# exoclime/HELIOS

Hardware: AMD Instinct MI355X
Metric: rad-conv iterations/sec x (lambda-bins x layers) (higher is better)
Workload: dtype f64; 1 GPU; BASELINE config 2: single column, 10 000 bins x 100 layers, premixed corr-k, isotropic scattering; nbin=10000, nlayer=100, ny=20, species=0, columns_per_gpu=1, columns_total=1, loop=radiative, parallelism=columns sharded, 1 per GPU

## Files before the change

helios_amd/csrc/rt_coef_kernel.inc:

```
template <int ROWS, int COEF_TPB>
__global__ void __launch_bounds__(64 * COEF_TPB) HX_COEF_KERNEL(KArgs a HX_PLANE_ARG) {
    using CT = HX_PLANE_T;
    extern __shared__ __align__(16) double smem[];
    const int col = blockIdx.y;
    if (a.done[col]) return;
    const int wave = threadIdx.x >> 6, lane = threadIdx.x & 63;
    const int ntiles = a.nblk_x * a.nparts * a.NW;
    const int TS = COEF_TPB * a.S;
    const int TSP = TS;
    const int NBX = a.coef_nbx;
    double* sh_lay = smem;
    double* sh_int = sh_lay + (size_t)a.L * TSP;
    double* sh_ray = sh_int + (size_t)a.I * TSP;
    double* sh_mu = sh_ray + (size_t)a.H * NBX;
    double* sh_dc = sh_mu + a.H;
    const size_t ncl = a.cloud_lds ? (size_t)a.H * NBX : 0;
    double* sh_g0 = sh_dc + a.H;
    double* sh_cab = sh_g0 + ncl;
    double* sh_csc = sh_cab + ncl;
    int* c_of_q = (int*)(sh_csc + ncl);
    int* x_of_q = c_of_q + TS;
    const size_t nc = (size_t)a.Y * a.X;
    const size_t wgI = nc * a.I;
    const int x_base = (blockIdx.x * COEF_TPB) / (a.NW * a.nparts) * a.nxb;
    for (int q = threadIdx.x; q < TS; q += blockDim.x) {
        const int tl = blockIdx.x * COEF_TPB + q / a.S, s_in_wave = q % a.S;
        int c = -1, xq = x_base;
        if (tl < ntiles) {
            const int wv = tl % a.NW, part = (tl / a.NW) % a.nparts, bx = tl / (a.NW * a.nparts);
            const int s_local = wv * a.S + s_in_wave;
            const int xl = s_local / a.ypb, yl = s_local - xl * a.ypb;
            const int x = bx * a.nxb + xl, y = part * a.ypb + yl;
            if (s_local < a.G && x < a.X) { c = y + a.Y * x; xq = x; }
        }
        c_of_q[q] = c;
        x_of_q[q] = xq;
    }
    {
        const double* mml = a.mmm_lay + (size_t)col * a.I;
        const double* mmi = a.mmm_int + (size_t)col * a.I;
        const double* dcu = a.dcol_u + (size_t)col * a.L;
        const double* dcl = a.dcol_l + (size_t)col * a.L;
        const double* pint = a.p_int + (size_t)col * a.I;
        const double grav = a.colpar[col].g;
        for (int h = threadIdx.x; h < a.H; h += blockDim.x) {
            if (a.iso) {
                sh_mu[h] = mml[h];
                sh_dc[h] = (pint[h] - pint[h + 1]) / grav;
            } else {
                const int i = h >> 1, ii = i + (h & 1);
                sh_mu[h] = (mmi[ii] + mml[i]) / 2.0;
                sh_dc[h] = (h & 1) ? dcu[i] : dcl[i];
            }
        }
        for (int t = threadIdx.x; t < a.H * NBX; t += blockDim.x) {
            const int xs = t / a.H, h = t - xs * a.H, x = min(x_base + xs, a.X - 1);
            const size_t src = ((size_t)col * a.X + x) * a.H + h;
            sh_ray[(size_t)h * NBX + xs] = a.half_ray[src];
            if (a.cloud_lds) {
                sh_g0[(size_t)h * NBX + xs] = a.half_g0[src];
                sh_cab[(size_t)h * NBX + xs] = a.half_cab[src];
                sh_csc[(size_t)h * NBX + xs] = a.half_csc[src];
            }
        }
    }
    __syncthreads();
    {
        const int q0 = threadIdx.x % TS, nrun = blockDim.x / TS, run = threadIdx.x / TS;
        const int cq = c_of_q[q0];
        if (a.from_table) {
            const size_t sp = nc, st = nc * a.npress;
            const double* ktable = a.coltab[col].k;
            for (int pass = 0; pass < (a.iso ? 1 : 2); pass++) {
                const int nlev = pass == 0 ? a.L : a.I;
                const TPIndex* tp = (pass == 0 ? a.tp_lay : a.tp_int) + (size_t)col * a.I;
                double* dst = pass == 0 ? sh_lay : sh_int;
                const int per = (nlev + nrun - 1) / nrun;
                const int l0 = run * per, l1 = min(nlev, l0 + per);
                int ktd = -1, ktu = -1, kpd = -1, kpu = -1;
                double c00 = 0, c01 = 0, c10 = 0, c11 = 0;
                TPIndex knext = tp[min(l0, nlev - 1)];
                for (int lev = l0; lev < l1; lev++) {
                    double v = 0.0;
                    const TPIndex k = knext;
                    knext = tp[min(lev + 1, nlev - 1)];
                    if (cq >= 0) {
                        if (k.tdown != ktd || k.tup != ktu || k.pdown != kpd || k.pup != kpu) {
                            const double* t0 = ktable + (size_t)cq + st * k.tdown;
                            const double* t1 = ktable + (size_t)cq + st * k.tup;
                            c00 = t0[sp * k.pdown];
                            c01 = t0[sp * k.pup];
                            c10 = t1[sp * k.pdown];
                            c11 = t1[sp * k.pup];
                            ktd = k.tdown; ktu = k.tup; kpd = k.pdown; kpu = k.pup;
                        }
                        v = blend_tp(c00, c01, c10, c11, k, false);
                    }
                    dst[(size_t)lev * TSP + q0] = v;
                }
            }
        } else {
            const double* opl = a.opac_wg_lay + col * wgI;
            const double* opi = a.opac_wg_int + col * wgI;
            for (int lev = run; lev < a.L; lev += nrun)
                sh_lay[(size_t)lev * TSP + q0] = cq >= 0 ? opl[(size_t)cq + nc * lev] : 0.0;
            if (!a.iso)
                for (int lev = run; lev < a.I; lev += nrun)
                    sh_int[(size_t)lev * TSP + q0] = cq >= 0 ? opi[(size_t)cq + nc * lev] : 0.0;
        }
    }
    __syncthreads();
    const int tl = blockIdx.x * COEF_TPB + wave;
    if (tl >= ntiles) return;
    const int j = lane % a.k, q = wave * a.S + lane / a.k;
    const int c = c_of_q[q], x = x_of_q[q], xs = x - x_base;
    const bool valid = c >= 0;
    const hx_rt_column cp = a.colpar[col];
    CT* ctile = HX_PLANES + col * a.coef_col + (size_t)tl * a.nplane * ROWS * 64;
    const double nmu = -cp.mu_star;
    const bool plain = a.clouds != 1 && a.scat_corr != 1 && a.g_0 == 0.0 && a.dir_beam != 1;
    const double* Fd = a.F_dir_wg + col * wgI;
    const double* Fc = a.Fc_dir_wg + col * wgI;
    auto beam_at_node = [&](int n) -> double {
        if (!(a.dir_beam == 1 && valid && n <= a.H)) return 0.0;
        if (a.iso) return Fd[(size_t)c + nc * n];
        return (n & 1) ? Fc[(size_t)c + nc * (n >> 1)] : Fd[(size_t)c + nc * (n >> 1)];
    };
    double F_here = beam_at_node(j * ROWS), F_above = beam_at_node(j * ROWS + 1);
    bool scatters = true;
    if (a.matrix) {
        bool mine = false;
#pragma unroll 1
        for (int r = 0; r < ROWS; r++) {
            const int h = j * ROWS + r;
            if (valid && h < a.H) {
                const int i = a.iso ? h : h >> 1;
                const bool lower = a.iso || (h & 1) == 0;
                const int ii = lower ? i : i + 1;
                double ray = 0.0, csc = 0.0, cab = 0.0;
                if (a.cloud_lds) {
                    cab = sh_cab[(size_t)h * NBX + xs];
                    csc = sh_csc[(size_t)h * NBX + xs];
                } else if (a.clouds == 1) {
                    const size_t src = ((size_t)col * a.X + x) * a.H + h;
                    cab = a.half_cab[src];
                    csc = a.half_csc[src];
                }
                if (a.scat == 1) ray = sh_ray[(size_t)h * NBX + xs];
                const double o_l = sh_lay[(size_t)i * TSP + q], o_i = a.iso ? o_l : sh_int[(size_t)ii * TSP + q];
                const double kap = a.iso ? o_l : (lower ? (o_i + o_l) / 2.0 : (o_l + o_i) / 2.0);
                mine = mine || single_scat_albedo(ray + csc, kap * sh_mu[h] + cab, a.w_0_limit) > a.w_0_scat_limit;
            }
        }
        const unsigned long long votes = __ballot(mine);
        const unsigned long long group = a.k >= 64 ? ~0ull : ((1ull << a.k) - 1ull) << (lane - j);
        scatters = (votes & group) != 0ull;
        if (valid && j == 0) a.trigger[col * nc + c] = scatters ? 1 : 0;
    }
    for (int r = 0; r < ROWS; r++) {
        const int h = j * ROWS + r;
        double alpha = 1.0, beta = 0.0, up = 0.0, vp = 0.0, dd = 0.0, du = 0.0;
        const double Fbot = F_here, Ftop = F_above;
        F_here = F_above;
        F_above = beam_at_node(h + 2);
        if (valid && h < a.H) {
            const int i = a.iso ? h : h >> 1;
            const bool lower = a.iso || (h & 1) == 0;
            const int ii = lower ? i : i + 1;
            double g0 = a.g_0, ray = 0.0, csc = 0.0, cab = 0.0;
            if (a.cloud_lds) {
                g0 = sh_g0[(size_t)h * NBX + xs];
                cab = sh_cab[(size_t)h * NBX + xs];
                csc = sh_csc[(size_t)h * NBX + xs];
            } else if (a.clouds == 1) {
                const size_t src = ((size_t)col * a.X + x) * a.H + h;
                g0 = a.half_g0[src];
                cab = a.half_cab[src];
                csc = a.half_csc[src];
            }
            if (a.scat == 1) ray = sh_ray[(size_t)h * NBX + xs];
            const double o_l = sh_lay[(size_t)i * TSP + q], o_i = a.iso ? o_l : sh_int[(size_t)ii * TSP + q];
            const double kap = a.iso ? o_l : (lower ? (o_i + o_l) / 2.0 : (o_l + o_i) / 2.0);
            const double mu = sh_mu[h], dcol = sh_dc[h];
            const double w0 = single_scat_albedo(ray + csc, kap * mu + cab, a.w_0_limit);
            const double dtau_gas = dcol * (kap + ray / mu);
            const double dtau = plain ? dtau_gas : dtau_gas + dcol * (cab + csc) / mu;
            const Slab s = plain ? slab_coeffs_plain(w0, dtau, a.epsi)
                                 : slab_coeffs(w0, dtau, g0, a.epsi, a.epsi2, cp.mu_star, a.scat_corr, a.i2s, a.dir_beam == 1);
            if (a.diag != nullptr && a.dir_beam == 1) {
                const int nlim = (fabs(s.Gp) >= 1e8 ? 1 : 0) + (fabs(s.Gm) >= 1e8 ? 1 : 0);
                if (nlim) atomicAdd(a.diag + HX_DIAG_G_LIMITED, (unsigned long long)nlim);
            }
            double invM = 1.0 / s.M;
            alpha = s.P * invM;
            beta = -s.N * invM;
            double K = 2.0 * HX_PI * a.epsi * (1.0 - w0) / (s.E - w0);
            double u, v;
            if (!scatters) {
                alpha = s.trans;
                beta = 0.0;
                invM = 1.0;
                K = 2.0 * HX_PI * a.epsi;
                if (a.iso || dtau < a.dtau_limit) {
                    u = v = (1.0 - s.trans) / 2.0;
                } else {
                    const double gq = a.epsi * (s.trans - 1.0) / dtau;
                    u = 1.0 + gq;
                    v = -s.trans - gq;
                }
            } else if (a.iso || dtau < a.dtau_limit) {
                u = v = (s.N + s.M - s.P) / 2.0;
            } else {
                const double qq = (plain ? a.epsi : a.epsi / (s.E * (1.0 - w0 * g0))) * (s.P - s.M + s.N) / dtau;
                u = (s.M + s.N) + qq;
                v = -s.P - qq;
            }
            up = K * u * invM;
            vp = K * v * invM;
            if (a.dir_beam == 1 && scatters) {
                const double dn = Fbot / nmu * (s.Gm * s.M + s.Gp * s.N) - Ftop / nmu * s.Gm * s.P;
                const double upw = Ftop / nmu * (s.Gm * s.N + s.Gp * s.M) - Fbot / nmu * s.P * s.Gp;
                dd = dmin(0.0, dn) * invM;
                du = dmin(0.0, upw) * invM;
            }
            if (h == 0) {
                a.boaK[col * nc + c] = scatters ? (1.0 - w0) / (s.E - w0) : 1.0;
                a.Fdir0[col * nc + c] = a.dir_beam == 1 ? (a.F_dir_wg + col * wgI)[c] : 0.0;
            }
        }
        const size_t off = plane_off(r, lane, ROWS);
        if constexpr (sizeof(CT) == sizeof(double)) {
            __builtin_nontemporal_store(alpha, ctile + 0 * ROWS * 64 + off);
            __builtin_nontemporal_store(beta, ctile + 1 * ROWS * 64 + off);
            __builtin_nontemporal_store(up, ctile + 2 * ROWS * 64 + off);
            if (a.has_vp) __builtin_nontemporal_store(vp, ctile + (size_t)a.pl_vp * ROWS * 64 + off);
        } else {
            __builtin_nontemporal_store(plane0_code(alpha, beta), ctile + 0 * ROWS * 64 + off);
            __builtin_nontemporal_store(plane1_code(beta), ctile + 1 * ROWS * 64 + off);
            __builtin_nontemporal_store((CT)up, ctile + 2 * ROWS * 64 + off);
            if (a.has_vp) __builtin_nontemporal_store((CT)(up + vp), ctile + (size_t)a.pl_vp * ROWS * 64 + off);
        }
        if (a.dir_beam == 1) {
            __builtin_nontemporal_store((CT)dd, ctile + (size_t)a.pl_dd * ROWS * 64 + off);
            __builtin_nontemporal_store((CT)du, ctile + (size_t)(a.pl_dd + 1) * ROWS * 64 + off);
        }
    }
}
```

helios_amd/csrc/rt_fused.h:

```cpp
#pragma once
#include <string>
#include <vector>

#include "hx_common.h"

namespace hx {

struct TileGeom {
    int k, ROWS, S;
    int nxb, ypb, nparts, G, NW, threads;
    int nblk_x;
    int nblk;
    int nplane;
    int has_vp, pl_vp, pl_dd;
    size_t tile_rows;
    size_t coef_elems_per_col, flux_elems_per_col;
};

struct Species {
    double* pretab = nullptr;
    double* scat_cross = nullptr;
    double* vmr_tab = nullptr;
    bool vmr_from_tab = false;
    double weight = 0.0;
    int is_h2o = 0, is_cia = 0, in_mu = 1;
    bool absorbing = false, scattering = false;
};

struct TableSet {
    const double *k, *scat_cross, *meanmass;
};

struct MieTable {
    const double *lam, *scat, *absorb;
    int nw, nr;
};

struct ProfileEntry {
    std::string name;
    hipEvent_t e0, e1;
};

}

struct hx_rt {
    hx_context* ctx;
    hx_rt_dims d;
    hx_rt_flags f;
    std::vector<hx_rt_column> cols;
    int X, Y, L, I, H, C, nsweep;
    hx::TileGeom g;
    bool have_grid = false, have_tables = false, have_planck = false, refreshed = false;
    bool keep_down = false;
    bool opac_stale = false;
    void* tp_lay = nullptr;
    void* tp_int = nullptr;
    double *T_lay_ref = nullptr, *T_int_ref = nullptr;
    int nchunk;
    int coef_tpb = 4;
    hipError_t shmem_rc = hipSuccess;
    bool cloud_lds = true;
    bool serpentine = false;
    unsigned flux_launches = 0;
    double state_cache_mb = 0;
    bool generic_scans = false;
    bool conv_shmem_raised = false;
    bool coef_shmem_raised = false;

    double *interwave = nullptr, *deltawave = nullptr, *wave = nullptr, *gauss_y = nullptr,
           *gauss_w = nullptr, *ktemp = nullptr, *kpress = nullptr;
    std::vector<hx::TableSet> tables;
    std::vector<int> col_table;
    hx::TableSet* coltab = nullptr;
    hx::TableSet* coltab_ref = nullptr;
    double* planck_grid = nullptr;
    std::vector<hx::Species> species;
    void* species_dev = nullptr;
    int* abs_list = nullptr;
    int nabs = 0;
    bool species_dev_stale = true;
    double *fac_lay = nullptr, *fac_int = nullptr;
    double *spec_lay = nullptr, *spec_int = nullptr;
    double *sc_spec_lay = nullptr, *sc_spec_int = nullptr;

    hx_rt_column* colpar = nullptr;
    double *p_lay = nullptr, *p_int = nullptr, *dcol_u = nullptr, *dcol_l = nullptr;
    double *T_lay = nullptr, *T_int = nullptr;
    double *surf_albedo = nullptr, *starflux = nullptr, *Bstar = nullptr;
    double *opac_wg_lay = nullptr, *opac_wg_int = nullptr;
    double *scat_cross_lay = nullptr, *scat_cross_int = nullptr;
    double *mmm_lay = nullptr, *mmm_int = nullptr;
    double *cl_abs_lay = nullptr, *cl_abs_int = nullptr, *cl_sc_lay = nullptr, *cl_sc_int = nullptr,
           *cl_g0_lay = nullptr, *cl_g0_int = nullptr, *g0_tot_lay = nullptr, *g0_tot_int = nullptr;
    double *half_ray = nullptr, *half_g0 = nullptr, *half_cab = nullptr, *half_csc = nullptr;
    double *vmr_lay = nullptr, *vmr_int = nullptr;
    double *delta_z = nullptr, *z_lay = nullptr;
    double *dtau_u = nullptr, *dtau_l = nullptr;
    double *F_dir_wg = nullptr, *Fc_dir_wg = nullptr;
    double* F_dir_band_n = nullptr;
    double* Bn = nullptr;
    double* coef = nullptr;
    float* coef32 = nullptr;
    int coef_bytes = 8;
    double* Utile = nullptr;
    double* Dtile = nullptr;
    double *U0 = nullptr, *boaK = nullptr, *Fdir0 = nullptr;
    double *F_down_band_n = nullptr, *F_up_band_n = nullptr;
    double* tot_part = nullptr;
    double *F_up_tot = nullptr, *F_down_tot = nullptr, *F_net = nullptr, *F_net_diff = nullptr;
    double *T_store = nullptr, *prefactor = nullptr;
    double *F_add_heat_lay = nullptr, *F_add_heat_sum = nullptr, *F_smooth = nullptr,
           *F_smooth_sum = nullptr, *c_p_lay = nullptr;
    int *abort_flags = nullptr, *conv_count = nullptr, *done = nullptr, *iters_done = nullptr;
    double *kappa_lay = nullptr, *kappa_int = nullptr, *dampara = nullptr;
    int *conv_unstable = nullptr, *conv_layer = nullptr, *marked_red = nullptr;
    double *entr_temp = nullptr, *entr_press = nullptr, *entr_kappa = nullptr, *entr_c_p = nullptr;
    int entr_ntemp = 0, entr_npress = 0;
    double* add_heat_dens = nullptr;
    bool has_heating = false;

    std::vector<hx::MieTable> mie;
    hx::MieTable* mie_dev = nullptr;
    double* cloud_spec = nullptr;
    int cloud_ndecks = 0;
    double* cloud_stage = nullptr;
    int* cloud_stage_index = nullptr;
    int cloud_stage_nr = 0;

    bool matrix = false;
    int* trigger = nullptr;
    bool matrix_keep_state = false;
    int* zero_flags = nullptr;
    int* iter_dev = nullptr;
    int iter_dev_expected = -1;
    hipGraphExec_t iter_graph = nullptr;
    hipGraphExec_t decade_graph = nullptr;
    long long iter_graph_replays = 0, decade_graph_replays = 0;
    long long iter_graph_builds = 0, decade_graph_builds = 0;
    long long graph_gen = 1, iter_graph_gen = 0, decade_graph_gen = 0;
    long long solve_serial = 1, matrix_tiles_serial = 0;
    int use_graph = -1;
    std::vector<char> have_albedo;

    bool profiling = false;
    std::vector<hx::ProfileEntry> prof;
    std::vector<std::pair<std::string, std::pair<double, int>>> prof_acc;
    std::vector<void*> allocs;
};
```

helios_amd/csrc/rt_fused.hip:

```cpp
#include "rt_kernels.h"
#include "rt_species.h"

#include <algorithm>
#include <cmath>

using namespace hx;

namespace {

int rt_fail(hx_rt* rt, int code, const char* msg) { return hx_fail(rt->ctx, code, "%s", msg); }

template <class T>
int dev_alloc(hx_rt* rt, T** p, size_t n, bool zero = true) {
    void* q = nullptr;
    if (n == 0) n = 1;
    hipError_t e = hipMalloc(&q, n * sizeof(T));
    if (e != hipSuccess)
        return hx_fail(rt->ctx, -(int)e, "hipMalloc of %zu bytes failed: %s", n * sizeof(T),
                       hipGetErrorString(e));
    if (zero) {
        e = hipMemsetAsync(q, 0, n * sizeof(T), rt->ctx->stream);
        if (e != hipSuccess) return hx_fail(rt->ctx, -(int)e, "hipMemset failed");
    }
    rt->allocs.push_back(q);
// ... 118 lines not shown
    a.U0 = rt->U0; a.boaK = rt->boaK; a.Fdir0 = rt->Fdir0;
    a.dtau_u = rt->dtau_u; a.dtau_l = rt->dtau_l;
    a.F_down_band_n = rt->F_down_band_n; a.F_up_band_n = rt->F_up_band_n; a.tot_part = rt->tot_part;
    a.F_up_tot = rt->F_up_tot; a.F_down_tot = rt->F_down_tot; a.F_net = rt->F_net;
    a.coef_col = g.coef_elems_per_col; a.flux_col = g.flux_elems_per_col;
    a.done = rt->done;
    a.coltab = rt->coltab; a.ktemp = rt->ktemp; a.kpress = rt->kpress;
    a.tp_lay = (const TPIndex*)rt->tp_lay; a.tp_int = (const TPIndex*)rt->tp_int;
    a.ntemp = rt->d.ntemp; a.npress = rt->d.npress; a.from_table = 0;
    a.iter_dev = rt->iter_dev;
    return a;
}

struct ProfScope {
    hx_rt* rt;
    hipEvent_t e0 = nullptr, e1 = nullptr;
    const char* name;
    ProfScope(hx_rt* r, const char* n) : rt(r), name(n) {
        if (!rt->profiling) return;
        (void)hipEventCreate(&e0);
        (void)hipEventCreate(&e1);
        (void)hipEventRecord(e0, rt->ctx->stream);
    }
    ~ProfScope() {
        if (!rt->profiling) return;
        (void)hipEventRecord(e1, rt->ctx->stream);
        rt->prof.push_back({name, e0, e1});
        if (rt->prof.size() > 8192) flush(rt);
    }
    static void flush(hx_rt* rt) {
        for (auto& p : rt->prof) {
            (void)hipEventSynchronize(p.e1);
            float ms = 0;
            (void)hipEventElapsedTime(&ms, p.e0, p.e1);
            bool found = false;
            for (auto& acc : rt->prof_acc)
                if (acc.first == p.name) {
                    acc.second.first += ms;
                    acc.second.second += 1;
                    found = true;
                }
            if (!found) rt->prof_acc.push_back({p.name, {ms, 1}});
            (void)hipEventDestroy(p.e0);
            (void)hipEventDestroy(p.e1);
        }
        rt->prof.clear();
    }
};

size_t flux_shmem_bytes(hx_rt* rt) {
    const TileGeom& g = rt->g;
    return ((size_t)g.nxb * (rt->H + 3) + (size_t)g.nxb * 2 * rt->I + (size_t)g.ypb * g.nxb * 2 * rt->I) *
           sizeof(double);
}

#define DISPATCH_ROWS(fn, rt, a)                  \
    switch ((rt)->g.ROWS) {                       \
        case 1: fn<1>(rt, a); break;              \
        case 2: fn<2>(rt, a); break;              \
        case 3: fn<3>(rt, a); break;              \
        case 4: fn<4>(rt, a); break;              \
        case 5: fn<5>(rt, a); break;              \
        case 6: fn<6>(rt, a); break;              \
        case 7: fn<7>(rt, a); break;              \
        case 8: fn<8>(rt, a); break;              \
        case 9: fn<9>(rt, a); break;              \
        case 10: fn<10>(rt, a); break;            \
        case 11: fn<11>(rt, a); break;            \
        case 12: fn<12>(rt, a); break;            \
        case 13: fn<13>(rt, a); break;            \
        case 14: fn<14>(rt, a); break;            \
        case 15: fn<15>(rt, a); break;            \
        case 20: fn<20>(rt, a); break;            \
        case 24: fn<24>(rt, a); break;            \
        case 28: fn<28>(rt, a); break;            \
        case 32: fn<32>(rt, a); break;            \
        default: fn<16>(rt, a); break;            \
    }

template <int ROWS, int K, bool MATRIX>
void flux_kernel(hx_rt* rt, const FluxArgs* f) {
    const size_t shmem = flux_shmem_bytes(rt);
    if (!f) {
        rt->shmem_rc = hipFuncSetAttribute((const void*)k_rt_flux<ROWS, K, MATRIX>, hipFuncAttributeMaxDynamicSharedMemorySize,
                                           (int)shmem);
        return;
    }
    hipLaunchKernelGGL(HIP_KERNEL_NAME(k_rt_flux<ROWS, K, MATRIX>), dim3(rt->g.nblk_x, rt->C), dim3(rt->g.threads), shmem,
                       rt->ctx->stream, *f);
}

template <int ROWS, bool MATRIX>
void flux_method(hx_rt* rt, const FluxArgs* f) {
    const int k = rt->g.k;
    const bool generic = rt->generic_scans;
    if constexpr (ROWS > 16) {
        (void)k; (void)generic;
        flux_kernel<ROWS, 64, MATRIX>(rt, f);
    } else {
        if (k == 16 && !generic) flux_kernel<ROWS, 16, MATRIX>(rt, f);
        else if (k == 32 && !generic) flux_kernel<ROWS, 32, MATRIX>(rt, f);
        else if (k == 64 && !generic) flux_kernel<ROWS, 64, MATRIX>(rt, f);
        else flux_kernel<ROWS, 0, MATRIX>(rt, f);
    }
}

template <int ROWS>
void flux_rows(hx_rt* rt, const FluxArgs* f) {
    if (rt->matrix) flux_method<ROWS, true>(rt, f);
    else flux_method<ROWS, false>(rt, f);
}

void launch_flux(hx_rt* rt, const KArgs& a) {
    const TileGeom& g = rt->g;
    FluxArgs f;
    memset(&f, 0, sizeof(f));
    f.X = a.X; f.Y = a.Y; f.L = a.L; f.I = a.I; f.H = a.H;
    f.k = a.k; f.nxb = a.nxb; f.ypb = a.ypb; f.nparts = a.nparts; f.G = a.G; f.NW = a.NW;
    f.dir_beam = a.dir_beam; f.nsweep = a.nsweep; f.keep_down = a.keep_down; f.has_vp = a.has_vp;
    f.pl_vp = a.pl_vp; f.pl_dd = a.pl_dd; f.nplane = a.nplane; f.iso = a.iso;
#ifdef HX_PROFILING
    static const int debug_skip = [] { const char* e = getenv("HELIOS_RT_DEBUG_SKIP"); return e ? atoi(e) : 0; }();
    f.debug_skip = debug_skip;
#endif
    f.Kconst = a.Kconst;
    f.trigger = a.trigger;
    f.keep_up = rt->matrix_keep_state ? 1 : 0;
    f.colpar = a.colpar;
    f.Bn = a.Bn; f.coef = a.coef; f.U0_in = a.U0; f.boaK = a.boaK; f.Fdir0 = a.Fdir0;
    f.surf_albedo = a.surf_albedo; f.gauss_w = a.gauss_w;
    f.Utile = a.Utile; f.Dtile = a.Dtile; f.U0 = a.U0; f.F_down_band_n = a.F_down_band_n;
    f.F_up_band_n = a.F_up_band_n;
    f.coef_col = a.coef_col; f.flux_col = a.flux_col;
    f.done = a.done;
    f.reverse = rt->serpentine ? (rt->flux_launches++ & 1) : 0;
    f.cache_state_from = INT_MAX;
    if (rt->serpentine && rt->state_cache_mb > 0) {
        const double per_wg = (double)g.nparts * g.NW * g.ROWS * 64 * sizeof(double);
        const long long total = (long long)g.nblk_x * rt->C;
        const long long keep = (long long)(rt->state_cache_mb * 1048576.0 / per_wg);
        f.cache_state_from = (int)std::max(0LL, total - keep);
    }
    if (rt->matrix) {
        f.reverse = 0;
        f.cache_state_from = INT_MAX;
    }
    if (rt->coef32) {
        launch_flux_f32(rt, f, dim3(g.nblk_x, rt->C), flux_shmem_bytes(rt));
        return;
    }
    DISPATCH_ROWS(flux_rows, rt, &f);
}

template <int ROWS, int TPB>
void launch_coef_tpb(hx_rt* rt, KArgs a) {
    const TileGeom& g = rt->g;
    const int ntiles = g.nblk_x * g.nparts * g.NW;
    const int TS = TPB * g.S, TSP = TS;
    const int NBX = g.nxb * ((TPB - 1) / (g.NW * g.nparts) + 2);
    a.coef_nbx = NBX;
    size_t shmem = ((size_t)(rt->L + rt->I) * TSP + (size_t)rt->H * (NBX + 2)) * sizeof(double) + 2 * TS * sizeof(int);
    const size_t cloud_image = 3 * (size_t)rt->H * NBX * sizeof(double);
    a.cloud_lds = a.clouds == 1 && rt->cloud_lds && shmem + cloud_image <= 80 * 1024;
    if (a.cloud_lds) shmem += cloud_image;
    if (rt->coef32) {
        launch_coef_f32(rt, a, TPB, dim3((ntiles + TPB - 1) / TPB, rt->C), shmem);
        return;
    }
    if (shmem > 64 * 1024 && !rt->coef_shmem_raised) {
        (void)hipFuncSetAttribute((const void*)k_rt_coef<ROWS, TPB>, hipFuncAttributeMaxDynamicSharedMemorySize,
                                  (int)shmem);
        rt->coef_shmem_raised = true;
    }
    hipLaunchKernelGGL(HIP_KERNEL_NAME(k_rt_coef<ROWS, TPB>), dim3((ntiles + TPB - 1) / TPB, rt->C), dim3(64 * TPB),
                       shmem, rt->ctx->stream, a);
}
template <int ROWS>
void launch_coef(hx_rt* rt, const KArgs& a) {
    switch (rt->coef_tpb) {
        case 1: launch_coef_tpb<ROWS, 1>(rt, a); break;
        case 2: launch_coef_tpb<ROWS, 2>(rt, a); break;
        case 8:
            if constexpr (ROWS <= 16) { launch_coef_tpb<ROWS, 8>(rt, a); break; }
            [[fallthrough]];
        default: launch_coef_tpb<ROWS, 4>(rt, a); break;
    }
}

size_t coef_shmem_bytes(const hx_rt* rt, int tpb) {
    const TileGeom& g = rt->g;
    const int TS = tpb * g.S;
    const int NBX = g.nxb * ((tpb - 1) / (g.NW * g.nparts) + 2);
    return ((size_t)(rt->L + rt->I) * TS + (size_t)rt->H * (NBX + 2)) * sizeof(double) + 2 * TS * sizeof(int);
}

int set_flux_shmem_limits(hx_rt* rt) {
    const size_t shmem = flux_shmem_bytes(rt);
    if (shmem > 160 * 1024) return rt_fail(rt, HX_E_UNSUPPORTED, "workgroup LDS demand exceeds 160 KiB");
    if (shmem <= 64 * 1024) return 0;
    if (rt->coef_bytes == 4) {
        HX_HIP(rt->ctx, raise_flux_shmem_f32(rt, (int)shmem));
        return 0;
    }
    DISPATCH_ROWS(flux_rows, rt, nullptr);
    HX_HIP(rt->ctx, rt->shmem_rc);
    return 0;
}

}

extern "C" {

int hx_rt_struct_sizes(int* dims_size, int* flags_size, int* column_size) {
    if (dims_size) *dims_size = (int)sizeof(hx_rt_dims);
    if (flags_size) *flags_size = (int)sizeof(hx_rt_flags);
    if (column_size) *column_size = (int)sizeof(hx_rt_column);
    return 0;
}

static int rt_create_into(hx_rt* rt, hx_context* ctx, const hx_rt_dims* dims, const hx_rt_flags* flags,
                          const hx_rt_column* columns);

int hx_rt_create(hx_context* ctx, const hx_rt_dims* dims, const hx_rt_flags* flags,
                 const hx_rt_column* columns, hx_rt** out_rt) {
    if (!ctx || !dims || !flags || !columns || !out_rt) return HX_E_ARG;
    *out_rt = nullptr;
    HX_REQUIRE(ctx, dims->nbin > 0 && dims->ny > 0 && dims->nlayer >= 1 && dims->ncol > 0, HX_E_ARG,
               "bad dimensions");
    HX_REQUIRE(ctx, dims->plancktable_dim >= 10 && dims->plancktable_step > 0, HX_E_ARG,
               "bad Planck-table dimensions");
    HX_HIP(ctx, hipSetDevice(ctx->device));
    hx_rt* rt = new hx_rt();
    const int rc_create = rt_create_into(rt, ctx, dims, flags, columns);
    if (rc_create) {
        hx_rt_destroy(rt);
        return rc_create;
    }
    *out_rt = rt;
    return 0;
}

static int rt_create_into(hx_rt* rt, hx_context* ctx, const hx_rt_dims* dims, const hx_rt_flags* flags,
                          const hx_rt_column* columns) {
    rt->ctx = ctx;
    rt->d = *dims;
    rt->f = *flags;
    rt->cols.assign(columns, columns + dims->ncol);
    rt->X = dims->nbin; rt->Y = dims->ny; rt->L = dims->nlayer; rt->I = rt->L + 1;
    rt->H = flags->iso ? rt->L : 2 * rt->L;
    rt->C = dims->ncol;
    rt->have_albedo.assign(dims->ncol, 0);
    rt->col_table.assign(dims->ncol, 0);
    RT_ALLOC(rt->iter_dev, 2);
    rt->nsweep = (flags->singlewalk ? 1000 : 3) * (flags->scat ? 1 : 0) + 1;
#ifdef HX_PROFILING
    if (const char* e = getenv("HELIOS_RT_DEBUG_NSWEEP")) rt->nsweep = atoi(e);
#endif
    if (const char* e = getenv("HELIOS_RT_MATRIX"))
        return hx_fail(ctx, HX_E_ARG, "HELIOS_RT_MATRIX=%s: the knob is retired (the matrix method has one solver); unset it", e);
    rt->matrix = flags->matrix != 0;
    rt->matrix_keep_state = rt->matrix && flags->debug == 1;
    if (!choose_geometry(rt->H, rt->Y, rt->X, rt->C, flags->dir_beam, flags->scat_corr, rt->g, rt->matrix ? 1 : 0))
        return hx_fail(ctx, HX_E_UNSUPPORTED, "fused path supports nlayer <= 1024 (2048 isothermal layers); use the per-stage API");
    rt->nchunk = std::max(1, std::min(512, std::max((rt->X + 47) / 48, std::min(32, (rt->X + 7) / 8))));
    if (const char* e = getenv("HELIOS_RT_GENERIC_SCANS")) rt->generic_scans = atoi(e) != 0;
    rt->coef_bytes = flags->coef_fp32 && !rt->matrix && coef_fp32_tiling(rt->g.ROWS, rt->g.k, rt->generic_scans) ? 4 : 8;
    if (const char* e = getenv("HELIOS_RT_CLOUD_LDS")) rt->cloud_lds = atoi(e) != 0;
    rt->coef_tpb = std::max(1, std::min(8, 16 / std::max(1, rt->g.S)));
    if (const char* e = getenv("HELIOS_RT_COEF_TPB")) rt->coef_tpb = atoi(e);
    if (rt->coef_tpb != 1 && rt->coef_tpb != 2 && !(rt->coef_tpb == 8 && rt->g.ROWS <= 16)) rt->coef_tpb = 4;
    while (rt->coef_tpb > 1 && coef_shmem_bytes(rt, rt->coef_tpb) > 150 * 1024) rt->coef_tpb /= 2;
    if (coef_shmem_bytes(rt, rt->coef_tpb) > 160 * 1024)
        return hx_fail(ctx, HX_E_UNSUPPORTED, "k_rt_coef's staging of one tile exceeds the 160 KiB of LDS");
    if (const char* e = getenv("HELIOS_RT_NCHUNK")) rt->nchunk = std::max(1, std::min(4096, atoi(e)));
    {
        const double state_mb = (double)rt->C * rt->g.flux_elems_per_col * sizeof(double) / 1048576.0;
        const double between_mb = (double)rt->C * rt->X * ((rt->H + 3) + 4.0 * rt->I) * sizeof(double) / 1048576.0;
        rt->serpentine = state_mb >= 64.0 && between_mb <= 64.0;
        rt->state_cache_mb = rt->serpentine ? 240.0 : 0.0;
    }
    if (const char* e = getenv("HELIOS_RT_SERPENTINE")) rt->serpentine = atoi(e) != 0;
    if (const char* e = getenv("HELIOS_RT_STATE_CACHE_MB")) rt->state_cache_mb = atof(e);
    rt->species.resize(dims->nspecies > 0 ? dims->nspecies : 0);
    int rc = set_flux_shmem_limits(rt);
    if (rc) return rc;

    const size_t X = rt->X, Y = rt->Y, L = rt->L, I = rt->I, C = rt->C, nc = X * Y;
    RT_ALLOC(rt->interwave, X + 1); RT_ALLOC(rt->deltawave, X); RT_ALLOC(rt->wave, X);
    RT_ALLOC(rt->gauss_y, Y); RT_ALLOC(rt->gauss_w, Y);
    RT_ALLOC(rt->ktemp, dims->ntemp); RT_ALLOC(rt->kpress, dims->npress);
    RT_ALLOC(rt->planck_grid, (size_t)(dims->plancktable_dim + 1) * X);
    RT_ALLOC(rt->colpar, C);
    RT_ALLOC(rt->coltab, C);
    RT_ALLOC(rt->coltab_ref, C);
    RT_ALLOC(rt->p_lay, C * L); RT_ALLOC(rt->p_int, C * I); RT_ALLOC(rt->dcol_u, C * L);
    RT_ALLOC(rt->dcol_l, C * L); RT_ALLOC(rt->T_lay, C * (L + 1)); RT_ALLOC(rt->T_int, C * I);
    RT_ALLOC(rt->surf_albedo, C * X); RT_ALLOC(rt->starflux, C * X); RT_ALLOC(rt->Bstar, C * X);
    RT_ALLOC(rt->opac_wg_lay, C * nc * I); RT_ALLOC(rt->opac_wg_int, C * nc * I);
    RT_ALLOC(rt->scat_cross_lay, C * X * I); RT_ALLOC(rt->scat_cross_int, C * X * I);
    RT_ALLOC(rt->mmm_lay, C * I); RT_ALLOC(rt->mmm_int, C * I);
    RT_ALLOC(rt->cl_abs_lay, C * X * I); RT_ALLOC(rt->cl_abs_int, C * X * I);
    RT_ALLOC(rt->cl_sc_lay, C * X * I); RT_ALLOC(rt->cl_sc_int, C * X * I);
    if (flags->clouds) {
        RT_ALLOC(rt->cl_g0_lay, C * X * I); RT_ALLOC(rt->cl_g0_int, C * X * I);
    }
    RT_ALLOC(rt->g0_tot_lay, C * X * I); RT_ALLOC(rt->g0_tot_int, C * X * I);
    RT_ALLOC(rt->half_ray, C * X * rt->H);
    if (flags->clouds) {
        RT_ALLOC(rt->half_g0, C * X * rt->H); RT_ALLOC(rt->half_cab, C * X * rt->H); RT_ALLOC(rt->half_csc, C * X * rt->H);
    }
    if (dims->nspecies > 0) {
        RT_ALLOC(rt->vmr_lay, C * dims->nspecies * I); RT_ALLOC(rt->vmr_int, C * dims->nspecies * I);
        RT_ALLOC(rt->spec_lay, nc * I); RT_ALLOC(rt->spec_int, nc * I);
        RT_ALLOC(rt->sc_spec_lay, X * I); RT_ALLOC(rt->sc_spec_int, X * I);
    }
    RT_ALLOC(rt->delta_z, C * L); RT_ALLOC(rt->z_lay, C * L);
    if (flags->dir_beam) {
        RT_ALLOC(rt->dtau_u, C * nc * L); RT_ALLOC(rt->dtau_l, C * nc * L);
        RT_ALLOC(rt->F_dir_wg, C * nc * I); RT_ALLOC(rt->Fc_dir_wg, C * nc * I);
    }
    RT_ALLOC(rt->F_dir_band_n, C * X * I);
    RT_ALLOC(rt->Bn, C * X * (rt->H + 3));
    if (rt->matrix) RT_ALLOC(rt->trigger, C * nc);
    if (rt->coef_bytes == 4) RT_ALLOC(rt->coef32, C * rt->g.coef_elems_per_col);
    else RT_ALLOC(rt->coef, C * rt->g.coef_elems_per_col);
    RT_ALLOC(rt->Utile, C * rt->g.flux_elems_per_col);
    RT_ALLOC(rt->U0, C * nc); RT_ALLOC(rt->boaK, C * nc); RT_ALLOC(rt->Fdir0, C * nc);
    RT_ALLOC(rt->F_down_band_n, C * X * I); RT_ALLOC(rt->F_up_band_n, C * X * I);
    RT_ALLOC(rt->tot_part, C * rt->nchunk * 2 * I);
    RT_ALLOC(rt->F_up_tot, C * I); RT_ALLOC(rt->F_down_tot, C * I); RT_ALLOC(rt->F_net, C * I);
    RT_ALLOC(rt->F_net_diff, C * L);
    RT_ALLOC(rt->T_store, C * (L + 1)); RT_ALLOC(rt->prefactor, C * (L + 1));
    RT_ALLOC(rt->F_add_heat_lay, C * L); RT_ALLOC(rt->F_add_heat_sum, C * L);
    RT_ALLOC(rt->F_smooth, C * L); RT_ALLOC(rt->F_smooth_sum, C * L); RT_ALLOC(rt->c_p_lay, C * L);
    RT_ALLOC(rt->abort_flags, C * (L + 1)); RT_ALLOC(rt->conv_count, C); RT_ALLOC(rt->done, C);
    RT_ALLOC(rt->kappa_lay, C * L); RT_ALLOC(rt->kappa_int, C * I); RT_ALLOC(rt->dampara, C);
    RT_ALLOC(rt->conv_unstable, C * (L + 1)); RT_ALLOC(rt->conv_layer, C * (L + 1)); RT_ALLOC(rt->marked_red, C * (L + 1));
    RT_ALLOC(rt->iters_done, C);
    {
        TPIndex* t1 = nullptr; TPIndex* t2 = nullptr;
        RT_ALLOC(t1, C * I); RT_ALLOC(t2, C * I);
        rt->tp_lay = t1; rt->tp_int = t2;
    }
    RT_ALLOC(rt->T_lay_ref, C * (L + 1)); RT_ALLOC(rt->T_int_ref, C * I);
    if (dims->nspecies > 0) {
        SpeciesDev* sd = nullptr;
        RT_ALLOC(sd, (size_t)dims->nspecies);
        rt->species_dev = sd;
        RT_ALLOC(rt->abs_list, (size_t)dims->nspecies);
        RT_ALLOC(rt->fac_lay, C * I * dims->nspecies); RT_ALLOC(rt->fac_int, C * I * dims->nspecies);
    }
    return h2d(rt, rt->colpar, rt->cols.data(), C * sizeof(hx_rt_column));
}

int hx_rt_destroy(hx_rt* rt) {
    if (!rt) return 0;
    if (rt->ctx) (void)hipStreamSynchronize(rt->ctx->stream);
    ProfScope::flush(rt);
    if (rt->iter_graph) (void)hipGraphExecDestroy(rt->iter_graph);
    if (rt->decade_graph) (void)hipGraphExecDestroy(rt->decade_graph);
    for (void* p : rt->allocs) (void)hipFree(p);
    delete rt;
    return 0;
}

#define RT_NEED_LOOP(rt)                                                                                             \
    do {                                                                                                             \
        if ((rt)->L < 2)                                                                                             \
            return hx_fail((rt)->ctx, HX_E_UNSUPPORTED, "%s: the batch has %d layer; refresh and iterations need at " \
                           "least 2", __func__, (rt)->L);                                                            \
    } while (0)

static inline void rt_touch(hx_rt* rt) {
    rt->graph_gen++;
    rt->solve_serial++;
}

int hx_rt_set_grid(hx_rt* rt, const double* opac_interwave, const double* opac_deltawave,
                   const double* opac_wave, const double* gauss_y, const double* gauss_weight,
                   const double* ktemp, const double* kpress) {
    if (!rt) return HX_E_ARG;
    rt_touch(rt);
    int rc = 0;
    rc |= h2d(rt, rt->interwave, opac_interwave, (rt->X + 1) * 8);
    rc |= h2d(rt, rt->deltawave, opac_deltawave, rt->X * 8);
    rc |= h2d(rt, rt->wave, opac_wave, rt->X * 8);
    rc |= h2d(rt, rt->gauss_y, gauss_y, rt->Y * 8);
    rc |= h2d(rt, rt->gauss_w, gauss_weight, rt->Y * 8);
    rc |= h2d(rt, rt->ktemp, ktemp, rt->d.ntemp * 8);
    rc |= h2d(rt, rt->kpress, kpress, rt->d.npress * 8);
    rt->have_grid = rc == 0;
    return rc;
}

static int for_cols(hx_rt* rt, int col, int* c0, int* c1);

static int upload_coltab(hx_rt* rt, int c0, int c1) {
    std::vector<TableSet> m(c1 - c0);
    for (int c = c0; c < c1; c++) m[c - c0] = rt->tables[rt->col_table[c]];
    return h2d(rt, rt->coltab + c0, m.data(), m.size() * sizeof(TableSet));
}

static int new_table_set(hx_rt* rt) {
    const size_t ntp = (size_t)rt->d.ntemp * rt->d.npress;
    const size_t n[3] = {ntp * rt->X * rt->Y, ntp * rt->X, ntp};
    double* p[3] = {nullptr, nullptr, nullptr};
    for (int i = 0; i < 3; i++)
        if (const int rc = dev_alloc(rt, &p[i], n[i])) {
            const std::string why = rt->ctx->err;
            return hx_fail(rt->ctx, rc, "premixed table set %d: %zu sets of %zu bytes each were asked for on this "
                           "device, the last one did not fit (%s)", (int)rt->tables.size(), rt->tables.size() + 1,
                           (n[0] + n[1] + n[2]) * 8, why.c_str());
        }
    rt->tables.push_back({p[0], p[1], p[2]});
    return rt->tables.size() == 1 ? upload_coltab(rt, 0, rt->C) : 0;
}

int hx_rt_set_premixed_tables(hx_rt* rt, const double* opac_k, const double* opac_scat_cross,
                              const double* opac_meanmass) {
    if (!rt) return HX_E_ARG;
    rt_touch(rt);
    HX_REQUIRE(rt->ctx, rt->d.nspecies == 0, HX_E_STATE, "object was created for on-the-fly mixing");
    const size_t ntp = (size_t)rt->d.ntemp * rt->d.npress;
    if (rt->tables.empty()) {
        int rc0 = new_table_set(rt);
        if (rc0) return rc0;
    }
    const TableSet& t = rt->tables[0];
    int rc = 0;
    rc |= h2d(rt, (void*)t.k, opac_k, ntp * rt->X * rt->Y * 8);
    rc |= h2d(rt, (void*)t.scat_cross, opac_scat_cross, ntp * rt->X * 8);
    rc |= h2d(rt, (void*)t.meanmass, opac_meanmass, ntp * 8);
    rt->have_tables = rc == 0;
    return rc;
}

int hx_rt_add_premixed_tables(hx_rt* rt, const double* opac_k, const double* opac_scat_cross, const double* opac_meanmass,
                              int* out_index) {
// ... 242 lines not shown
}

int hx_rt_set_convergence_limit(hx_rt* rt, int col, double limit) {
    if (!rt) return HX_E_ARG;
    rt_touch(rt);
    int c0, c1, rc = for_cols(rt, col, &c0, &c1);
    if (rc) return rc;
    for (int c = c0; c < c1; c++) {
        rt->cols[c].rad_convergence_limit = limit;
        rc |= h2d(rt, &rt->colpar[c], &rt->cols[c], sizeof(hx_rt_column));
    }
    return rc;
}


int hx_rt_build_planck_table(hx_rt* rt, int energy_correction) {
    if (!rt) return HX_E_ARG;
    rt_touch(rt);
    HX_REQUIRE(rt->ctx, rt->have_grid, HX_E_STATE, "hx_rt_set_grid first");
    hx_context* ctx = rt->ctx;
    const int X = rt->X, dim = rt->d.plancktable_dim, step = rt->d.plancktable_step;
    int rc = hx_plancktable(ctx, rt->planck_grid, rt->interwave, rt->deltawave, X, rt->cols[0].T_star,
                            dim, step);
    if (rc) return rc;
    for (int c = 0; c < rt->C; c++) {
        const double Ts = rt->cols[c].T_star;
        double* brow = rt->Bstar + (size_t)c * X;
        double* sflux = rt->starflux + (size_t)c * X;
        rc = hx_internal_planck_star_row(ctx, brow, rt->interwave, rt->deltawave, X, Ts);
        if (rc) return rc;
        if (energy_correction == 1 && Ts > 10) {
            rc = hx_corr_inc_energy(ctx, brow, sflux, rt->deltawave, rt->f.real_star, X, Ts, 0);
            if (rc) return rc;
        }
        if (rt->f.real_star == 1) {
            std::vector<double> tmp(X);
            rc = hx_d2h(ctx, tmp.data(), sflux, X * 8);
            if (rc) return rc;
            for (auto& v : tmp) v = v / HX_PI;
            rc = h2d(rt, brow, tmp.data(), X * 8);
            if (rc) return rc;
        }
        if (c == 0) {
            rc = hx_d2d(ctx, rt->planck_grid + (size_t)dim * X, brow, X * 8);
            if (rc) return rc;
        }
    }
    rt->have_planck = true;
    return 0;
}

static int upload_species_table(hx_rt* rt) {
    if (!rt->species_dev_stale) return 0;
    const int S = rt->d.nspecies;
    std::vector<SpeciesDev> sd(S);
    std::vector<int> abs;
    for (int s = 0; s < S; s++) {
        const Species& sp = rt->species[s];
        sd[s] = SpeciesDev{sp.pretab, sp.scat_cross, sp.vmr_from_tab ? sp.vmr_tab : nullptr, sp.weight, sp.absorbing ? 1 : 0,
                           sp.scattering ? 1 : 0,
                           sp.is_h2o ? 1 : 0, (rt->f.kcoeff_mixing_ro && !sp.is_cia && rt->Y != 1) ? 1 : 0,
                           sp.in_mu, 0};
        if (sp.absorbing) abs.push_back(s);
    }
    int rc = h2d(rt, rt->species_dev, sd.data(), S * sizeof(SpeciesDev));
    if (!rc && !abs.empty()) rc = h2d(rt, rt->abs_list, abs.data(), abs.size() * sizeof(int));
    rt->nabs = (int)abs.size();
    rt->species_dev_stale = rc != 0;
    return rc;
}

extern "C++" int hx::launch_mix_species(hx_context* ctx, MixArgs m, const int* abs_list, int nabs_all) {
    const long long npair = (long long)m.C * (m.L + m.I) * m.X;
    if (npair <= 0) return 0;
    static const int waves = [] { const char* e = getenv("HELIOS_RT_MIX_WAVES"); return e ? atoi(e) : 256 * 16 * 48; }();
    const int grid = (int)std::min(npair, (long long)waves);
    static const int extra_lds = [] { const char* e = getenv("HELIOS_RT_MIX_EXTRA_LDS"); return e ? atoi(e) : 0; }();
    for (int first = 0; first == 0 || first < nabs_all; first += MIX_MAX_ABSORBERS) {
        m.abs_list = abs_list + first;
        m.nabs = std::min(MIX_MAX_ABSORBERS, nabs_all - first);
        m.carry_on = first > 0 ? 1 : 0;
        k_rt_mix_species<<<grid, 64, extra_lds, ctx->stream>>>(m);
        HX_LAUNCH_CHECK(ctx);
    }
    return 0;
}

static int refresh_species(hx_rt* rt) {
    hx_context* ctx = rt->ctx;
    int rc = upload_species_table(rt);
    if (rc) return rc;
    MixArgs m;
    m.X = rt->X; m.Y = rt->Y; m.L = rt->L; m.I = rt->I; m.C = rt->C; m.S = rt->d.nspecies;
    m.ntemp = rt->d.ntemp; m.npress = rt->d.npress; m.nabs = rt->nabs; m.carry_on = 0;
    m.sp = (const SpeciesDev*)rt->species_dev; m.abs_list = rt->abs_list;
    m.T_lay = rt->T_lay; m.T_int = rt->T_int; m.p_lay = rt->p_lay; m.p_int = rt->p_int;
    m.vmr_lay = rt->vmr_lay; m.vmr_int = rt->vmr_int;
    m.ktemp = rt->ktemp; m.kpress = rt->kpress; m.gauss_w = rt->gauss_w; m.gauss_y = rt->gauss_y; m.wave = rt->wave;
    m.mmm_lay = rt->mmm_lay; m.mmm_int = rt->mmm_int;
    m.tp_lay = (TPIndex*)rt->tp_lay; m.tp_int = (TPIndex*)rt->tp_int;
    m.fac_lay = rt->fac_lay; m.fac_int = rt->fac_int;
    m.opac_wg_lay = rt->opac_wg_lay; m.opac_wg_int = rt->opac_wg_int;
    m.scat_lay = rt->scat_cross_lay; m.scat_int = rt->scat_cross_int;
    m.done = rt->done; m.diag = ctx->diag;
    k_rt_species_prep<<<dim3(hx_cdiv(rt->I, 64), rt->C), 64, 0, ctx->stream>>>(m);
    HX_LAUNCH_CHECK(ctx);
    {
        ProfScope ps(rt, "add_to_mixed_opac");
        rc = launch_mix_species(ctx, m, rt->abs_list, rt->nabs);
        if (rc) return rc;
    }
    {
        ProfScope ps(rt, "mixed_scat");
        k_rt_scat_species<<<dim3(hx_cdiv(rt->X, 256), rt->L + rt->I, rt->C), 256, 0, ctx->stream>>>(m);
        HX_LAUNCH_CHECK(ctx);
    }
    return 0;
}

int hx_rt_refresh(hx_rt* rt) {
    if (!rt) return HX_E_ARG;
    RT_NEED_LOOP(rt);
    hx_context* ctx = rt->ctx;
    rt->solve_serial++;
    HX_REQUIRE(ctx, rt->have_grid && rt->have_tables && rt->have_planck, HX_E_STATE,
               "set grid, tables and build the Planck table first");
    HX_REQUIRE(ctx, !rt->matrix || std::all_of(rt->have_albedo.begin(), rt->have_albedo.end(), [](char v) { return v != 0; }),
               HX_E_STATE, "the matrix method needs a surface albedo (> 0) for every column of the batch");
    const int X = rt->X, Y = rt->Y, L = rt->L, I = rt->I, C = rt->C;
    const size_t nc = (size_t)X * Y;
    int rc = 0;
    if (rt->d.nspecies > 0) {
        bool any_ro = false;
        for (const Species& sp : rt->species) any_ro = any_ro || (sp.absorbing && rt->f.kcoeff_mixing_ro && !sp.is_cia);
        if (Y != ro::NY && Y != 1 && any_ro)
            return hx_fail(ctx, HX_E_RO_NY, "random-overlap mixing needs ny == 20 or 1 (got %d)", Y);
        HX_REQUIRE(ctx, Y <= ro::NY, HX_E_UNSUPPORTED, "on-the-fly mixing in the fused path holds at most 20 Gauss points");
        int nabs = 0;
        for (const Species& sp : rt->species) nabs += sp.absorbing ? 1 : 0;
        (void)nabs;
    }
    KArgs a = make_args(rt);
    rt->iter_dev_expected = -1;
    {
        ProfScope ps(rt, "rt_nodes");
        dim3 grid(hx_cdiv(X, 32), hx_cdiv(rt->H + 3, 32), C);
        k_rt_nodes<<<grid, 256, 0, ctx->stream>>>(a);
        HX_LAUNCH_CHECK(ctx);
    }
    ProfScope ps_all(rt, "refresh_total");
    bool fused_lookup = rt->d.nspecies == 0 && !rt->f.dir_beam;
    if (const char* e = getenv("HELIOS_RT_FUSED_LOOKUP")) fused_lookup = fused_lookup && atoi(e) != 0;
    rt->opac_stale = fused_lookup;
    if (rt->d.nspecies == 0) {
        k_rt_tp_index<<<dim3(hx_cdiv(I, 64), C), 64, 0, ctx->stream>>>(a, (TPIndex*)rt->tp_lay, (TPIndex*)rt->tp_int);
        k_rt_scat_interp<<<dim3(hx_cdiv(X, 256), I, C), 256, 0, ctx->stream>>>(a, rt->scat_cross_lay, rt->scat_cross_int);
        k_rt_mmm_table<<<dim3(hx_cdiv(I, 64), C), 64, 0, ctx->stream>>>(a, rt->mmm_lay, rt->mmm_int);
        HX_LAUNCH_CHECK(ctx);
        if (fused_lookup) {
            k_rt_keep_ref_T<<<dim3(hx_cdiv(I + 1, 64), C), 64, 0, ctx->stream>>>(a, rt->T_lay_ref, rt->T_int_ref, rt->coltab_ref);
        } else {
            ProfScope ps(rt, "opac_interpol");
            const int chunks = (int)std::min<long long>(hx_cdiv((long long)nc, 256), 1024);
            k_rt_opac_table<<<dim3(chunks, I, C), 256, 0, ctx->stream>>>(a, rt->opac_wg_lay, rt->opac_wg_int);
        }
        HX_LAUNCH_CHECK(ctx);
    } else {
        rc = refresh_species(rt);
        if (rc) return rc;
    }
    if (rt->f.clouds) {
        k_rt_total_g0<<<dim3(hx_cdiv(X, 256), I, C), 256, 0, ctx->stream>>>(a, rt->cl_g0_lay, rt->cl_g0_int,
                                                                          rt->g0_tot_lay, rt->g0_tot_int);
        HX_LAUNCH_CHECK(ctx);
    }
    k_rt_delta_z<<<dim3(hx_cdiv(L, 64), C), 64, 0, ctx->stream>>>(a, rt->delta_z);
    k_rt_height<<<C, 64, 0, ctx->stream>>>(rt->p_lay, rt->delta_z, rt->z_lay, L, rt->f.planet_type_gas, (size_t)L, rt->done);
    HX_LAUNCH_CHECK(ctx);
    if (rt->has_heating) {
        k_rt_heating<<<C, 64, 0, ctx->stream>>>(rt->add_heat_dens, rt->delta_z, rt->F_add_heat_lay,
                                                rt->F_add_heat_sum, L, rt->done);
        HX_LAUNCH_CHECK(ctx);
    }
    if (rt->f.dir_beam) {
        ProfScope ps(rt, "direct_beam");
        k_rt_dtau_halves<<<dim3(hx_cdiv((long long)nc, 256), L, C), 256, 0, ctx->stream>>>(a);
        HX_LAUNCH_CHECK(ctx);
        rc = hx_internal_fdir_noniso_batch(ctx, rt->F_dir_wg, rt->f.iso ? nullptr : rt->Fc_dir_wg, rt->Bstar, rt->dtau_u, rt->dtau_l,
                                           rt->z_lay, rt->colpar, rt->done, C, rt->f.dir_beam,
                                           rt->f.geom_zenith_corr, I, X, Y);
        if (rc) return rc;
        k_rt_fdir_band<<<dim3(hx_cdiv(X, 32), hx_cdiv(I, 32), C), 256, 0, ctx->stream>>>(rt->F_dir_wg, rt->F_dir_band_n,
                                                                           rt->gauss_w, X, Y, I, rt->done);
        HX_LAUNCH_CHECK(ctx);
    }
    {
        ProfScope ps(rt, "rt_coef");
        k_rt_half_bands<<<dim3(hx_cdiv(X, 32), hx_cdiv(rt->H, 32), C), 256, 0, ctx->stream>>>(a);
        HX_LAUNCH_CHECK(ctx);
        a.from_table = fused_lookup ? 1 : 0;
        DISPATCH_ROWS(launch_coef, rt, a);
        HX_LAUNCH_CHECK(ctx);
    }
    rt->refreshed = true;
    return 0;
}

namespace { int kappa_cp_from_table(hx_rt* rt, bool refresh_T_int); }

static int count_negative_fluxes(hx_rt* rt) {
    const size_t n = (size_t)rt->C * rt->g.flux_elems_per_col;
    int rc = hx_internal_count_negative(rt->ctx, rt->Utile, n, HX_DIAG_NEG_UP);
    if (!rc && rt->keep_down && rt->Dtile) rc = hx_internal_count_negative(rt->ctx, rt->Dtile, n, HX_DIAG_NEG_DOWN);
    return rc;
}

static int spectral_fluxes(hx_rt* rt, const KArgs& a) {
    {
        ProfScope ps(rt, rt->matrix ? "matrix_solve" : "rt_flux");
        launch_flux(rt, a);
        HX_LAUNCH_CHECK(rt->ctx);
    }
    return rt->f.debug == 1 ? count_negative_fluxes(rt) : 0;
}

static int rt_step_kernels(hx_rt* rt, int itervalue, int step_temperature, bool nodes_done) {
    hx_context* ctx = rt->ctx;
    rt->solve_serial++;
    KArgs a = make_args(rt);
    if (!nodes_done) {
        ProfScope ps(rt, "rt_nodes");
        dim3 grid(hx_cdiv(rt->X, 32), hx_cdiv(rt->H + 3, 32), rt->C);
        k_rt_nodes<<<grid, 256, 0, ctx->stream>>>(a);
        HX_LAUNCH_CHECK(ctx);
    }
    {
        int rc = spectral_fluxes(rt, a);
        if (rc) return rc;
    }
    {
        ProfScope ps(rt, "rt_totals_a");
        k_rt_totals_a<<<dim3(rt->nchunk, rt->C), 256, 0, ctx->stream>>>(a);
        HX_LAUNCH_CHECK(ctx);
    }
    if (rt->entr_kappa && rt->cols[0].physical_tstep != 0 && itervalue % 10 == 0) {
        int rc = kappa_cp_from_table(rt, false);
        if (rc) return rc;
    }
    {
        ProfScope ps(rt, "rt_totals_b");
        TotalsBArgs q;
        q.a = a;
        memset(&q.rt, 0, sizeof(q.rt));
        q.rt.F_net_diff = rt->F_net_diff;
        q.rt.tlay = rt->T_lay;
        q.rt.play = rt->p_lay;
        q.rt.pint = rt->p_int;
        q.rt.abrt = rt->abort_flags;
        q.rt.T_store = rt->T_store;
        q.rt.deltat_prefactor = rt->prefactor;
        q.rt.F_add_heat_lay = rt->F_add_heat_lay;
        q.rt.F_add_heat_sum = rt->F_add_heat_sum;
        q.rt.F_smooth = rt->F_smooth;
        q.rt.F_smooth_sum = rt->F_smooth_sum;
        q.rt.c_p_lay = rt->c_p_lay;
        q.rt.conv_count = rt->conv_count;
        q.rt.itervalue = itervalue;
        q.rt.nlayer = rt->L;
        q.rt.smooth = rt->f.smooth;
        q.rt.dim = rt->d.plancktable_dim;
        q.rt.step = rt->d.plancktable_step;
        q.step_temperature = step_temperature;
        q.done_w = rt->done;
        q.iters_done = rt->iters_done;
        q.iter_dev = rt->iter_dev;
        k_rt_totals_b<<<rt->C, 1024, 0, ctx->stream>>>(q);
        HX_LAUNCH_CHECK(ctx);
    }
    return 0;
}

__global__ void k_rt_set_iteration(int* iter_dev, int next) { iter_dev[0] = next; }

static int sync_iteration_counter(hx_rt* rt, int itervalue) {
    if (rt->iter_dev_expected == itervalue) return 0;
    k_rt_set_iteration<<<1, 1, 0, rt->ctx->stream>>>(rt->iter_dev, itervalue);
    HX_LAUNCH_CHECK(rt->ctx);
    rt->iter_dev_expected = itervalue;
    return 0;
}

int hx_rt_step(hx_rt* rt, int itervalue, int step_temperature) {
    if (!rt) return HX_E_ARG;
    RT_NEED_LOOP(rt);
    int rc = sync_iteration_counter(rt, itervalue);
    if (rc) return rc;
    bool nodes_done = false;
    if (itervalue % 10 == 0 || !rt->refreshed) {
        rc = hx_rt_refresh(rt);
        if (rc) return rc;
        nodes_done = true;
    }
    rc = rt_step_kernels(rt, itervalue, step_temperature, nodes_done);
    rt->iter_dev_expected = rc ? -1 : itervalue + 1;
    return rc;
}

namespace {

ConvKArgs make_conv_args(hx_rt* rt, int itervalue) {
    ConvKArgs c;
    memset(&c, 0, sizeof(c));
    c.L = rt->L; c.C = rt->C; c.itervalue = itervalue;
    c.colpar = rt->colpar;
    c.T_lay = rt->T_lay; c.p_lay = rt->p_lay; c.p_int = rt->p_int;
    c.kappa_lay = rt->kappa_lay; c.kappa_int = rt->kappa_int;
    c.c_p = rt->c_p_lay; c.mmm_lay = rt->mmm_lay;
    c.F_add_heat_sum = rt->F_add_heat_sum; c.F_smooth_sum = rt->F_smooth_sum;
    c.F_down_tot = rt->F_down_tot; c.F_up_tot = rt->F_up_tot; c.F_net = rt->F_net;
    c.conv_unstable = rt->conv_unstable; c.conv_layer = rt->conv_layer; c.marked_red = rt->marked_red;
    c.dampara = rt->dampara;
    c.done = rt->done;
    return c;
}

}

namespace {

int kappa_cp_from_table(hx_rt* rt, bool refresh_T_int) {
    hx_context* ctx = rt->ctx;
    const int L = rt->L, I = rt->I;
    if (refresh_T_int) {
        k_rt_tint<<<dim3(hx_cdiv(I, 64), rt->C), 64, 0, ctx->stream>>>(rt->T_lay, rt->T_int, L, rt->done);
        HX_LAUNCH_CHECK(ctx);
    }
    for (int c = 0; c < rt->C; c++) {
        const double* T_lay = rt->T_lay + (size_t)c * (L + 1);
        const double* T_int = rt->T_int + (size_t)c * I;
        const double* p_lay = rt->p_lay + (size_t)c * L;
        const double* p_int = rt->p_int + (size_t)c * I;
        int rc = hx_kappa_interpol(ctx, T_lay, rt->entr_temp, p_lay, rt->entr_press, rt->kappa_lay + (size_t)c * L,
                                   rt->entr_kappa, rt->entr_npress, rt->entr_ntemp, L);
        if (rc) return rc;
        rc = hx_kappa_interpol(ctx, T_int, rt->entr_temp, p_int, rt->entr_press, rt->kappa_int + (size_t)c * I,
                               rt->entr_kappa, rt->entr_npress, rt->entr_ntemp, I);
        if (rc) return rc;
        rc = hx_cp_interpol(ctx, T_lay, rt->entr_temp, p_lay, rt->entr_press, rt->c_p_lay + (size_t)c * L,
                            rt->entr_c_p, rt->entr_npress, rt->entr_ntemp, L);
        if (rc) return rc;
    }
    return 0;
}

// ... 158 lines not shown
        rc = hx_rt_refresh(rt);
        if (!rc) rc = rt_step_kernels(rt, 1, 1, true);
    }
    for (int n = 0; n < GRAPH_ITERATIONS && !rc; n++) rc = rt_step_kernels(rt, 1, 1, false);
    hipGraph_t graph = nullptr;
    const hipError_t e = hipStreamEndCapture(ctx->stream, &graph);
    if (rc || e != hipSuccess || !graph) {
        if (graph) (void)hipGraphDestroy(graph);
        rt->use_graph = 0;
        (void)hipGetLastError();
        return 0;
    }
    const hipError_t ei = hipGraphInstantiate(&exec, graph, nullptr, nullptr, 0);
    (void)hipGraphDestroy(graph);
    if (ei != hipSuccess) {
        exec = nullptr;
        rt->use_graph = 0;
        (void)hipGetLastError();
        return 0;
    }
    (with_refresh ? rt->decade_graph_gen : rt->iter_graph_gen) = rt->graph_gen;
    (with_refresh ? rt->decade_graph_builds : rt->iter_graph_builds)++;
    return 0;
}

int hx_rt_run(hx_rt* rt, int itervalue, int nsteps) {
    if (!rt) return HX_E_ARG;
    RT_NEED_LOOP(rt);
    for (int n = 0; n < nsteps;) {
        const int it = itervalue + n;
        const bool decade = it % 10 == 0 && nsteps - n >= GRAPH_ITERATIONS + 1 && (rt->d.nspecies == 0 || !rt->species_dev_stale);
        if ((decade || (it % 10 == 1 && nsteps - n >= GRAPH_ITERATIONS)) && rt->refreshed && graph_wanted(rt)) {
            hipGraphExec_t& exec = decade ? rt->decade_graph : rt->iter_graph;
            if ((decade ? rt->decade_graph_gen : rt->iter_graph_gen) != rt->graph_gen || !exec) {
                int rc = build_iteration_graph(rt, decade);
                if (rc) return rc;
            }
            if (exec) {
                int rc = sync_iteration_counter(rt, it);
                if (rc) return rc;
                HX_HIP(rt->ctx, hipGraphLaunch(exec, rt->ctx->stream));
                rt->solve_serial++;
                (decade ? rt->decade_graph_replays : rt->iter_graph_replays)++;
                const int done = GRAPH_ITERATIONS + (decade ? 1 : 0);
                rt->iter_dev_expected = it + done;
                n += done;
                continue;
            }
        }
        int rc = hx_rt_step(rt, it, 1);
        if (rc) return rc;
        n++;
    }
    return 0;
}

int hx_rt_converged_layers(hx_rt* rt, int* out_counts) {
    if (!rt) return HX_E_ARG;
    return hx_d2h(rt->ctx, out_counts, rt->conv_count, rt->C * sizeof(int));
}

namespace {

int get_plain(hx_rt* rt, const void* dptr, size_t bytes, void* out, size_t out_bytes) {
    if (bytes != out_bytes)
        return hx_fail(rt->ctx, HX_E_ARG, "hx_rt_get: buffer is %zu bytes, array has %zu", out_bytes, bytes);
    return hx_d2h(rt->ctx, out, dptr, bytes);
}

int get_band(hx_rt* rt, const double* dptr, void* out, size_t out_bytes) {
    const size_t X = rt->X, I = rt->I;
    if (out_bytes != X * I * 8) return hx_fail(rt->ctx, HX_E_ARG, "hx_rt_get: wrong buffer size");
    std::vector<double> tmp(X * I);
    int rc = hx_d2h(rt->ctx, tmp.data(), dptr, X * I * 8);
    if (rc) return rc;
    double* o = (double*)out;
    for (size_t x = 0; x < X; x++)
        for (size_t i = 0; i < I; i++) o[x + X * i] = tmp[x * I + i];
    return 0;
}

int get_flux_wg(hx_rt* rt, int col, const double* tiles, const double* bc, bool up, bool interface_nodes,
                void* out, size_t out_bytes) {
    const TileGeom& g = rt->g;
    const size_t X = rt->X, Y = rt->Y, I = rt->I, nc = X * Y;
    if (out_bytes != nc * I * 8) return hx_fail(rt->ctx, HX_E_ARG, "hx_rt_get: wrong buffer size");
    std::vector<double> t(g.flux_elems_per_col), b(nc);
    int rc = hx_d2h(rt->ctx, t.data(), tiles + (size_t)col * g.flux_elems_per_col, t.size() * 8);
    if (rc) return rc;
    if (bc) {
        rc = hx_d2h(rt->ctx, b.data(), bc + (size_t)col * nc, nc * 8);
        if (rc) return rc;
    }
    double* o = (double*)out;
    std::fill(o, o + nc * I, 0.0);
    for (int blk = 0; blk < g.nblk; blk++) {
        const int bx = blk / g.nparts, part = blk % g.nparts;
        for (int s = 0; s < g.G; s++) {
            const int xl = s / g.ypb, yl = s % g.ypb;
            const size_t x = (size_t)bx * g.nxb + xl, y = (size_t)part * g.ypb + yl;
            if (x >= X) continue;
            const size_t c = y + Y * x;
            for (int j = 0; j < g.k; j++) {
                const int tid = s * g.k + j, wv = tid / 64, lane = tid % 64;
                const double* tile = t.data() + ((size_t)blk * g.NW + wv) * g.ROWS * 64;
                for (int r = 0; r < g.ROWS; r++) {
                    const int h = j * g.ROWS + r;
                    if (h >= rt->H) continue;
                    const int node = up ? h + 1 : h;
                    if (rt->f.iso) {
                        if (interface_nodes) o[c + nc * node] = tile[plane_off(r, lane, g.ROWS)];
                        continue;
                    }
                    const bool is_int = (node % 2) == 0;
                    if (is_int != interface_nodes) continue;
                    o[c + nc * (node / 2)] = tile[plane_off(r, lane, g.ROWS)];
                }
            }
            if (up && interface_nodes && bc) o[c] = b[c];
        }
    }
    return 0;
}

}

static int materialize_opac(hx_rt* rt) {
    if (!rt->opac_stale) return 0;
    hx_context* ctx = rt->ctx;
    const size_t nc = (size_t)rt->X * rt->Y, wgI = nc * rt->I, bandI = (size_t)rt->X * rt->I;
    std::vector<TableSet> used(rt->C);
    int rc0 = hx_d2h(ctx, used.data(), rt->coltab_ref, used.size() * sizeof(TableSet));
    if (rc0) return rc0;
    for (int c = 0; c < rt->C; c++) {
        const TableSet& t = used[c];
        int rc = hx_opac_interpol(ctx, rt->T_lay_ref + (size_t)c * (rt->L + 1), rt->ktemp, rt->p_lay + (size_t)c * rt->L,
                                  rt->kpress, t.k, rt->opac_wg_lay + c * wgI, t.scat_cross,
                                  rt->scat_cross_lay + c * bandI, rt->d.npress, rt->d.ntemp, rt->Y, rt->X, rt->L);
        if (rc) return rc;
        rc = hx_opac_interpol(ctx, rt->T_int_ref + (size_t)c * rt->I, rt->ktemp, rt->p_int + (size_t)c * rt->I,
                              rt->kpress, t.k, rt->opac_wg_int + c * wgI, t.scat_cross,
                              rt->scat_cross_int + c * bandI, rt->d.npress, rt->d.ntemp, rt->Y, rt->X, rt->I);
        if (rc) return rc;
    }
    rt->opac_stale = false;
    return 0;
}

int hx_rt_get(hx_rt* rt, int col, const char* name, void* out, size_t out_bytes) {
    if (!rt) return HX_E_ARG;
    if (strcmp(name, "coef_plane_bytes") == 0) {
        HX_REQUIRE(rt->ctx, out_bytes == sizeof(int32_t), HX_E_ARG, "coef_plane_bytes is one int32");
        const int32_t v = rt->coef_bytes;
        memcpy(out, &v, sizeof(v));
        return 0;
    }
    if (strcmp(name, "flux_tiling") == 0) {
        const TileGeom& g = rt->g;
        const int32_t v[14] = {g.k, g.ROWS, g.threads, g.nparts, g.nxb, g.ypb, g.NW, g.nplane, g.has_vp, g.pl_vp, g.pl_dd,
                               rt->coef_tpb, rt->coef_bytes, rt->generic_scans ? 1 : 0};
        HX_REQUIRE(rt->ctx, out_bytes == sizeof(v), HX_E_ARG, "flux_tiling is 14 int32");
        memcpy(out, v, sizeof(v));
        return 0;
    }
    if (strcmp(name, "premixed_table_count") == 0) {
        HX_REQUIRE(rt->ctx, out_bytes == sizeof(int32_t), HX_E_ARG, "premixed_table_count is one int32");
        const int32_t v = (int32_t)rt->tables.size();
        memcpy(out, &v, sizeof(v));
        return 0;
    }
    if (strcmp(name, "mie_table_count") == 0) {
        HX_REQUIRE(rt->ctx, out_bytes == sizeof(int32_t), HX_E_ARG, "mie_table_count is one int32");
        const int32_t v = (int32_t)rt->mie.size();
        memcpy(out, &v, sizeof(v));
        return 0;
    }
    HX_REQUIRE(rt->ctx, col >= 0 && col < rt->C, HX_E_ARG, "column index out of range");
    if (strcmp(name, "premixed_table") == 0) {
        HX_REQUIRE(rt->ctx, out_bytes == sizeof(int32_t), HX_E_ARG, "premixed_table is one int32");
        const int32_t v = rt->col_table[col];
        memcpy(out, &v, sizeof(v));
        return 0;
    }
    if (strcmp(name, "coef_planes") == 0) {
        const void* planes = rt->coef32 ? (const void*)rt->coef32 : (const void*)rt->coef;
        const size_t bytes = rt->g.coef_elems_per_col * rt->coef_bytes;
        return get_plain(rt, (const char*)planes + (size_t)col * bytes, bytes, out, out_bytes);
    }
    if (strncmp(name, "opac_wg_", 8) == 0) {
        int rc = materialize_opac(rt);
        if (rc) return rc;
    }
    const size_t X = rt->X, Y = rt->Y, L = rt->L, I = rt->I, nc = X * Y, c = col;
    const std::string n(name);
    if (n == "T_lay") return get_plain(rt, rt->T_lay + c * (L + 1), (L + 1) * 8, out, out_bytes);
    if (n == "T_int") return get_plain(rt, rt->T_int + c * I, I * 8, out, out_bytes);
    if (n == "F_up_band") return get_band(rt, rt->F_up_band_n + c * X * I, out, out_bytes);
    if (n == "F_down_band") return get_band(rt, rt->F_down_band_n + c * X * I, out, out_bytes);
    if (n == "F_dir_band") return get_band(rt, rt->F_dir_band_n + c * X * I, out, out_bytes);
    if (n == "F_up_tot") return get_plain(rt, rt->F_up_tot + c * I, I * 8, out, out_bytes);
    if (n == "F_down_tot") return get_plain(rt, rt->F_down_tot + c * I, I * 8, out, out_bytes);
    if (n == "F_net") return get_plain(rt, rt->F_net + c * I, I * 8, out, out_bytes);
    if (n == "F_net_diff") return get_plain(rt, rt->F_net_diff + c * L, L * 8, out, out_bytes);
    if (n == "abort") return get_plain(rt, rt->abort_flags + c * (L + 1), (L + 1) * 4, out, out_bytes);
    if (n == "delta_t_prefactor") return get_plain(rt, rt->prefactor + c * (L + 1), (L + 1) * 8, out, out_bytes);
    if (n == "T_store") return get_plain(rt, rt->T_store + c * (L + 1), (L + 1) * 8, out, out_bytes);
    if (n == "delta_z_lay") return get_plain(rt, rt->delta_z + c * L, L * 8, out, out_bytes);
    if (n == "z_lay") return get_plain(rt, rt->z_lay + c * L, L * 8, out, out_bytes);
    if (n == "meanmolmass_lay") return get_plain(rt, rt->mmm_lay + c * I, L * 8, out, out_bytes);
    if (n == "meanmolmass_int") return get_plain(rt, rt->mmm_int + c * I, I * 8, out, out_bytes);
    if (n == "opac_wg_lay") return get_plain(rt, rt->opac_wg_lay + c * nc * I, nc * L * 8, out, out_bytes);
    if (n == "opac_wg_int") return get_plain(rt, rt->opac_wg_int + c * nc * I, nc * I * 8, out, out_bytes);
    if (n == "scat_cross_lay") return get_plain(rt, rt->scat_cross_lay + c * X * I, X * L * 8, out, out_bytes);
    if (n == "scat_cross_int") return get_plain(rt, rt->scat_cross_int + c * X * I, X * I * 8, out, out_bytes);
    if (n == "abs_cross_all_clouds_lay") return get_plain(rt, rt->cl_abs_lay + c * X * I, X * L * 8, out, out_bytes);
    if (n == "abs_cross_all_clouds_int") return get_plain(rt, rt->cl_abs_int + c * X * I, X * I * 8, out, out_bytes);
    if (n == "scat_cross_all_clouds_lay") return get_plain(rt, rt->cl_sc_lay + c * X * I, X * L * 8, out, out_bytes);
    if (n == "scat_cross_all_clouds_int") return get_plain(rt, rt->cl_sc_int + c * X * I, X * I * 8, out, out_bytes);
    if (n == "g_0_all_clouds_lay" || n == "g_0_all_clouds_int") {
        HX_REQUIRE(rt->ctx, rt->f.clouds == 1, HX_E_STATE, "object was created with clouds = 0");
        return n == "g_0_all_clouds_lay" ? get_plain(rt, rt->cl_g0_lay + c * X * I, X * L * 8, out, out_bytes)
                                         : get_plain(rt, rt->cl_g0_int + c * X * I, X * I * 8, out, out_bytes);
    }
    if (n == "cloud_deck_spectra") {
        HX_REQUIRE(rt->ctx, rt->cloud_ndecks > 0, HX_E_STATE, "no cloud decks have been set (hx_rt_set_column_cloud_decks)");
        const size_t per = (size_t)rt->cloud_ndecks * 3 * X;
        return get_plain(rt, rt->cloud_spec + c * per, per * 8, out, out_bytes);
    }
    if (n == "g_0_tot_lay") return get_plain(rt, rt->g0_tot_lay + c * X * I, X * L * 8, out, out_bytes);
    if (n == "g_0_tot_int") return get_plain(rt, rt->g0_tot_int + c * X * I, X * I * 8, out, out_bytes);
    if ((n == "vmr_lay" || n == "vmr_int") && rt->d.nspecies > 0) {
        const size_t S = rt->d.nspecies;
        return get_plain(rt, (n == "vmr_lay" ? rt->vmr_lay : rt->vmr_int) + c * S * I, S * I * 8, out, out_bytes);
    }
    if (n == "iters_done") return get_plain(rt, rt->iters_done + c, 4, out, out_bytes);
    if (n == "flux_launch_policy") {
        HX_REQUIRE(rt->ctx, out_bytes == 2 * sizeof(double), HX_E_ARG, "flux_launch_policy is two doubles");
        const double v[2] = {rt->serpentine ? 1.0 : 0.0, rt->serpentine ? rt->state_cache_mb : 0.0};
        memcpy(out, v, sizeof(v));
        return 0;
    }
    if (n == "graph_replays") {
        HX_REQUIRE(rt->ctx, out_bytes == 3 * sizeof(double), HX_E_ARG, "graph_replays is three doubles");
        const double v[3] = {(double)rt->iter_graph_replays, (double)rt->decade_graph_replays, rt->use_graph == 1 ? 1.0 : 0.0};
        memcpy(out, v, sizeof(v));
        return 0;
    }
    if (n == "graph_builds") {
        HX_REQUIRE(rt->ctx, out_bytes == 2 * sizeof(double), HX_E_ARG, "graph_builds is two doubles");
        const double v[2] = {(double)rt->iter_graph_builds, (double)rt->decade_graph_builds};
        memcpy(out, v, sizeof(v));
        return 0;
    }
    if (n == "planck_grid")
        return get_plain(rt, rt->planck_grid, (size_t)(rt->d.plancktable_dim + 1) * X * 8, out, out_bytes);
    if (n == "done") return get_plain(rt, rt->done + c, 4, out, out_bytes);
    if (n == "conv_layer") return get_plain(rt, rt->conv_layer + c * (L + 1), (L + 1) * 4, out, out_bytes);
    if (n == "conv_unstable") return get_plain(rt, rt->conv_unstable + c * (L + 1), (L + 1) * 4, out, out_bytes);
    if (n == "marked_red") return get_plain(rt, rt->marked_red + c * (L + 1), (L + 1) * 4, out, out_bytes);
    if (n == "F_smooth_sum") return get_plain(rt, rt->F_smooth_sum + c * L, L * 8, out, out_bytes);
    if (n == "kappa_lay") return get_plain(rt, rt->kappa_lay + c * L, L * 8, out, out_bytes);
    if (n == "kappa_int") return get_plain(rt, rt->kappa_int + c * (L + 1), (L + 1) * 8, out, out_bytes);
    if (n == "c_p_lay") return get_plain(rt, rt->c_p_lay + c * L, L * 8, out, out_bytes);
    if (n == "F_add_heat_lay") return get_plain(rt, rt->F_add_heat_lay + c * L, L * 8, out, out_bytes);
    if (n == "F_add_heat_sum") return get_plain(rt, rt->F_add_heat_sum + c * L, L * 8, out, out_bytes);
    if (n == "planckband_lay" || n == "planckband_int") {
        const bool lay = n == "planckband_lay";
        const size_t NN = rt->H + 3, per = lay ? L + 2 : I;
        if (out_bytes != X * per * 8) return hx_fail(rt->ctx, HX_E_ARG, "hx_rt_get: wrong buffer size");
        std::vector<double> tmp(X * NN);
        int rc = hx_d2h(rt->ctx, tmp.data(), rt->Bn + c * X * NN, X * NN * 8);
        if (rc) return rc;
        double* o = (double*)out;
        for (size_t x = 0; x < X; x++) {
            if (lay) {
                for (size_t i = 0; i < L; i++) o[i + x * per] = tmp[x * NN + (rt->f.iso ? i : 2 * i + 1)];
                o[L + x * per] = tmp[x * NN + rt->H + 1];
                o[L + 1 + x * per] = tmp[x * NN + rt->H + 2];
            } else {
                for (size_t i = 0; i < I; i++) o[i + x * per] = rt->f.iso ? 0.0 : tmp[x * NN + 2 * i];
            }
        }
        return 0;
    }
    if (rt->matrix && (n == "F_up_wg" || n == "F_down_wg" || n == "Fc_up_wg" || n == "Fc_down_wg")) {
        HX_REQUIRE(rt->ctx, rt->refreshed, HX_E_STATE, "no iteration has been run yet");
        const bool first = !rt->Dtile;
        if (!rt->Dtile) RT_ALLOC(rt->Dtile, (size_t)rt->C * rt->g.flux_elems_per_col);
        if (!rt->zero_flags) RT_ALLOC(rt->zero_flags, (size_t)rt->C);
        if (first || rt->matrix_tiles_serial != rt->solve_serial) {
            const bool kd = rt->keep_down, ks = rt->matrix_keep_state;
            rt->keep_down = true;
            rt->matrix_keep_state = true;
            KArgs a = make_args(rt);
            a.done = rt->zero_flags;
            launch_flux(rt, a);
            rt->keep_down = kd;
            rt->matrix_keep_state = ks;
            HX_LAUNCH_CHECK(rt->ctx);
            rt->matrix_tiles_serial = rt->solve_serial;
        }
        if (first) rt->graph_gen++;
    }
    if (n == "F_up_wg") return get_flux_wg(rt, col, rt->Utile, rt->U0, true, true, out, out_bytes);
    if (n == "Fc_up_wg") return get_flux_wg(rt, col, rt->Utile, nullptr, true, false, out, out_bytes);
    if (n == "F_down_wg" || n == "Fc_down_wg") {
// ... 199 lines not shown
```

helios_amd/csrc/rt_fused_f32.hip:

```cpp
#define HX_PLANE_KERNELS_ONLY
#include "rt_kernels.h"

using namespace hx;

namespace hx {

bool coef_fp32_tiling(int rows, int k, bool generic_scans) {
    return rows <= 13 || (rows == 14 && k == 16 && !generic_scans);
}

namespace {

template <int ROWS, int TPB>
void coef_tpb(hx_rt* rt, const KArgs& a, dim3 grid, size_t shmem) {
    if (shmem > 64 * 1024 && !rt->coef_shmem_raised) {
        (void)hipFuncSetAttribute((const void*)k_rt_coef_f32<ROWS, TPB>, hipFuncAttributeMaxDynamicSharedMemorySize,
                                  (int)shmem);
        rt->coef_shmem_raised = true;
    }
    hipLaunchKernelGGL(HIP_KERNEL_NAME(k_rt_coef_f32<ROWS, TPB>), grid, dim3(64 * TPB), shmem, rt->ctx->stream, a,
                       rt->coef32);
}

template <int ROWS>
void coef_rows(hx_rt* rt, const KArgs& a, int tpb, dim3 grid, size_t shmem) {
    switch (tpb) {
        case 1: coef_tpb<ROWS, 1>(rt, a, grid, shmem); break;
        case 2: coef_tpb<ROWS, 2>(rt, a, grid, shmem); break;
        case 8: coef_tpb<ROWS, 8>(rt, a, grid, shmem); break;
        default: coef_tpb<ROWS, 4>(rt, a, grid, shmem); break;
    }
}

template <int ROWS, int K, bool MATRIX>
hipError_t flux_kernel(hx_rt* rt, const FluxArgs* f, dim3 grid, size_t shmem, int raise) {
    if (raise)
        return hipFuncSetAttribute((const void*)k_rt_flux_f32<ROWS, K, MATRIX>, hipFuncAttributeMaxDynamicSharedMemorySize, raise);
    hipLaunchKernelGGL(HIP_KERNEL_NAME(k_rt_flux_f32<ROWS, K, MATRIX>), grid, dim3(rt->g.threads), shmem, rt->ctx->stream, *f,
                       (const float*)rt->coef32);
    return hipSuccess;
}

template <int ROWS, bool MATRIX>
hipError_t flux_method(hx_rt* rt, const FluxArgs* f, dim3 grid, size_t shmem, int raise) {
    const int k = rt->g.k;
    const bool generic = rt->generic_scans;
    if constexpr (ROWS == 14) {
        (void)k; (void)generic;
        return flux_kernel<14, 16, MATRIX>(rt, f, grid, shmem, raise);
    } else {
        if (k == 16 && !generic) return flux_kernel<ROWS, 16, MATRIX>(rt, f, grid, shmem, raise);
        if (k == 32 && !generic) return flux_kernel<ROWS, 32, MATRIX>(rt, f, grid, shmem, raise);
        if (k == 64 && !generic) return flux_kernel<ROWS, 64, MATRIX>(rt, f, grid, shmem, raise);
        return flux_kernel<ROWS, 0, MATRIX>(rt, f, grid, shmem, raise);
    }
}

template <int ROWS>
hipError_t flux_rows(hx_rt* rt, const FluxArgs* f, dim3 grid, size_t shmem, int raise) {
    return flux_method<ROWS, false>(rt, f, grid, shmem, raise);
}

#define F32_DISPATCH_ROWS(fn, ...)                          \
    switch (rt->g.ROWS) {                                   \
        case 1: return fn<1>(rt, __VA_ARGS__);              \
        case 2: return fn<2>(rt, __VA_ARGS__);              \
        case 3: return fn<3>(rt, __VA_ARGS__);              \
        case 4: return fn<4>(rt, __VA_ARGS__);              \
        case 5: return fn<5>(rt, __VA_ARGS__);              \
        case 6: return fn<6>(rt, __VA_ARGS__);              \
        case 7: return fn<7>(rt, __VA_ARGS__);              \
        case 8: return fn<8>(rt, __VA_ARGS__);              \
        case 9: return fn<9>(rt, __VA_ARGS__);              \
        case 10: return fn<10>(rt, __VA_ARGS__);            \
        case 11: return fn<11>(rt, __VA_ARGS__);            \
        case 12: return fn<12>(rt, __VA_ARGS__);            \
        case 13: return fn<13>(rt, __VA_ARGS__);            \
        default: return fn<14>(rt, __VA_ARGS__);            \
    }

}

void launch_coef_f32(hx_rt* rt, const KArgs& a, int tpb, dim3 grid, size_t shmem) {
    F32_DISPATCH_ROWS(coef_rows, a, tpb, grid, shmem);
}

void launch_flux_f32(hx_rt* rt, const FluxArgs& f, dim3 grid, size_t shmem) {
    (void)[&]() -> hipError_t { F32_DISPATCH_ROWS(flux_rows, &f, grid, shmem, 0); }();
}

hipError_t raise_flux_shmem_f32(hx_rt* rt, int shmem) {
    F32_DISPATCH_ROWS(flux_rows, nullptr, dim3(1), 0, shmem);
}

}
```

helios_amd/csrc/rt_kernels.h:

```cpp
#pragma once
#include "rt_fused.h"
#include "conv_adjust.h"
#include "temp_step.h"
#include "two_stream.h"
#include "plane_code.h"

namespace hx {

struct KArgs {
    int X, Y, L, I, H, C;
    int k, ROWS, S, nxb, ypb, nparts, G, NW, nblk_x, nblk, nplane, nchunk, coef_nbx;
    int cloud_lds;
    int scat, dir_beam, clouds, scat_corr, nsweep, keep_down, real_star;
    int iso;
    int has_vp, pl_vp, pl_dd;
    int matrix;
    int* trigger;
    double Kconst;
    int dim, step;
    double epsi, epsi2, g_0, i2s, w_0_limit, w_0_scat_limit, dtau_limit;
    const hx_rt_column* colpar;
    const double *T_lay, *p_lay, *p_int, *dcol_u, *dcol_l, *surf_albedo, *Bstar, *planck_grid;
    const double *opac_wg_lay, *opac_wg_int, *scat_cross_lay, *scat_cross_int, *mmm_lay, *mmm_int;
    const double *cl_abs_lay, *cl_abs_int, *cl_sc_lay, *cl_sc_int, *g0_tot_lay, *g0_tot_int;
// ... 175 lines not shown
        Bc = fma(A, B2, Bc);
        A *= A2;
    }
}
#undef HX_SCAN32_ROW_STEP

struct LaneMap {
    int lane, wv, j, x, y, xl, yl;
    bool valid;
    size_t sp;
    size_t tile;
};

__device__ __forceinline__ int opaque_tid() {
    int t = threadIdx.x;
    asm volatile("" : "+v"(t));
    return t;
}

template <class Args>
__device__ __forceinline__ LaneMap lane_map(const Args& a, int bx, int part, int tid) {
    LaneMap m;
    m.lane = tid & 63;
    m.wv = tid >> 6;
    m.j = m.lane & (a.k - 1);
    const int s_local = tid >> (31 - __clz(a.k));
    m.xl = s_local / a.ypb;
    m.yl = s_local - m.xl * a.ypb;
    m.x = bx * a.nxb + m.xl;
    m.y = part * a.ypb + m.yl;
    m.valid = s_local < a.G && m.x < a.X;
    m.sp = (size_t)m.y + (size_t)a.Y * m.x;
    m.tile = ((size_t)bx * a.nparts + part) * a.NW + m.wv;
    return m;
}

template <int CTRL>
__device__ __forceinline__ void compose_row_neighbour(double& A, double& Bc) {
    const int a_lo = __builtin_amdgcn_update_dpp(0, __double2loint(A), CTRL, 0xf, 0xf, true);
    const int a_hi = __builtin_amdgcn_update_dpp(0x3FF00000, __double2hiint(A), CTRL, 0xf, 0xf, false);
    const int b_lo = __builtin_amdgcn_update_dpp(0, __double2loint(Bc), CTRL, 0xf, 0xf, true);
    const int b_hi = __builtin_amdgcn_update_dpp(0, __double2hiint(Bc), CTRL, 0xf, 0xf, true);
    Bc = fma(A, __hiloint2double(b_hi, b_lo), Bc);
    A *= __hiloint2double(a_hi, a_lo);
}

template <int CTRL>
__device__ __forceinline__ double dpp_or_zero(double v) {
    const int lo = __builtin_amdgcn_update_dpp(0, __double2loint(v), CTRL, 0xf, 0xf, true);
    const int hi = __builtin_amdgcn_update_dpp(0, __double2hiint(v), CTRL, 0xf, 0xf, true);
    return __hiloint2double(hi, lo);
}

template <int SRC>
__device__ __forceinline__ double wave_lane(double v) {
    return __hiloint2double(__builtin_amdgcn_readlane(__double2hiint(v), SRC), __builtin_amdgcn_readlane(__double2loint(v), SRC));
}

template <int K>
__device__ __forceinline__ void scan_down_fixed(double& A, double& Bc, int j, int lane) {
    compose_row_neighbour<0x101>(A, Bc);
    compose_row_neighbour<0x102>(A, Bc);
    compose_row_neighbour<0x104>(A, Bc);
    compose_row_neighbour<0x108>(A, Bc);
    if (K == 32 || K == 64) {
        const double A2 = group_lane16(A, lane), B2 = group_lane16(Bc, lane);
        if ((lane & 16) == 0) {
            Bc = fma(A, B2, Bc);
            A *= A2;
        }
    }
    if (K == 64) {
        const double A2 = wave_lane<32>(A), B2 = wave_lane<32>(Bc);
        if (lane < 32) {
            Bc = fma(A, B2, Bc);
            A *= A2;
        }
    }
}
template <int K>
__device__ __forceinline__ void scan_up_fixed(double& A, double& Bc, int j) {
    compose_row_neighbour<0x111>(A, Bc);
    compose_row_neighbour<0x112>(A, Bc);
    compose_row_neighbour<0x114>(A, Bc);
    compose_row_neighbour<0x118>(A, Bc);
    if (K == 32 || K == 64) {
        const double A2 = dpp_move<0x142, 0xa>(A), B2 = dpp_move<0x142, 0xa>(Bc);
        if (j & 16) {
            Bc = fma(A, B2, Bc);
            A *= A2;
        }
    }
    if (K == 64) {
        const double A2 = dpp_move<0x143, 0xc>(A), B2 = dpp_move<0x143, 0xc>(Bc);
        if (j >= 32) {
            Bc = fma(A, B2, Bc);
            A *= A2;
        }
    }
}
template <int K>
__device__ __forceinline__ double below_fixed(double v) {
    return K == 16 ? dpp_or_zero<0x111>(v) : dpp_or_zero<0x138>(v);
}
template <int K>
__device__ __forceinline__ double above_fixed(double v) {
    return K == 16 ? dpp_or_zero<0x101>(v) : dpp_or_zero<0x130>(v);
}
template <int K>
__device__ __forceinline__ double group_first_lane(double v, int lane) {
    if (K == 16) return dpp_or_zero<0x150>(v);
    if (K == 64) return wave_lane<0>(v);
    const int lo = __double2loint(v), hi = __double2hiint(v);
    const int lo_a = __builtin_amdgcn_readlane(lo, 0), lo_b = __builtin_amdgcn_readlane(lo, 32);
    const int hi_a = __builtin_amdgcn_readlane(hi, 0), hi_b = __builtin_amdgcn_readlane(hi, 32);
    return __hiloint2double(lane < 32 ? hi_a : hi_b, lane < 32 ? lo_a : lo_b);
}
__device__ __forceinline__ double tiny_abs_below(double F, double thr) { return fabs(F) < thr ? fabs(F) : F; }

#ifndef HX_PLANE_KERNELS_ONLY
__global__ void __launch_bounds__(256) k_rt_half_bands(KArgs a) {
    __shared__ double tile[4][32][33];
    const int col = blockIdx.z;
    if (a.done[col]) return;
    const int tx = threadIdx.x & 31, ty = threadIdx.x >> 5;
    const size_t bandI = (size_t)a.X * a.I;
    const double* src_i[4] = {a.scat_cross_int + col * bandI, a.g0_tot_int + col * bandI, a.cl_abs_int + col * bandI,
                              a.cl_sc_int + col * bandI};
    const double* src_l[4] = {a.scat_cross_lay + col * bandI, a.g0_tot_lay + col * bandI, a.cl_abs_lay + col * bandI,
                              a.cl_sc_lay + col * bandI};
    double* dst[4] = {a.half_ray, a.half_g0, a.half_cab, a.half_csc};
    const int nq = a.clouds == 1 ? 4 : 1;
    const int x = blockIdx.x * 32 + tx;
    for (int hh = ty; hh < 32; hh += 8) {
        const int h = blockIdx.y * 32 + hh;
        if (x < a.X && h < a.H) {
            const int i = a.iso ? h : h >> 1, ii = a.iso ? h : i + (h & 1);
            const size_t b_l = x + (size_t)a.X * i, b_i = x + (size_t)a.X * ii;
            for (int q = 0; q < nq; q++) {
                const bool on = q == 1 || q == 2 || a.scat == 1;
                tile[q][hh][tx] = !on ? 0.0 : a.iso ? src_l[q][b_l] : (src_i[q][b_i] + src_l[q][b_l]) / 2.0;
            }
        }
    }
    __syncthreads();
    const int h = blockIdx.y * 32 + tx;
    for (int xx = ty; xx < 32; xx += 8) {
        const int xo = blockIdx.x * 32 + xx;
        if (xo < a.X && h < a.H)
            for (int q = 0; q < nq; q++) dst[q][((size_t)col * a.X + xo) * a.H + h] = tile[q][tx][xx];
    }
}

#endif

#define HX_COEF_KERNEL k_rt_coef
#define HX_PLANE_T double
#define HX_PLANE_ARG
#define HX_PLANES a.coef
#include "rt_coef_kernel.inc"
#undef HX_COEF_KERNEL
#undef HX_PLANE_T
#undef HX_PLANE_ARG
#undef HX_PLANES
#define HX_COEF_KERNEL k_rt_coef_f32
#define HX_PLANE_T float
#define HX_PLANE_ARG , float* coef32
#define HX_PLANES coef32
#include "rt_coef_kernel.inc"
#undef HX_COEF_KERNEL
#undef HX_PLANE_T
#undef HX_PLANE_ARG
#undef HX_PLANES

#ifndef HX_PLANE_KERNELS_ONLY
__global__ void __launch_bounds__(256) k_rt_dtau_halves(KArgs a) {
    const int col = blockIdx.z, i = blockIdx.y;
    const size_t nc = (size_t)a.Y * a.X;
    const size_t c = (size_t)blockIdx.x * blockDim.x + threadIdx.x;
    if (c >= nc || a.done[col]) return;
    const int x = (int)(c / a.Y);
    const size_t wgI = nc * a.I, bandI = (size_t)a.X * a.I;
    const double* opl = a.opac_wg_lay + col * wgI;
    const double* opi = a.opac_wg_int + col * wgI;
    const double* scl = a.scat_cross_lay + col * bandI;
    const double* sci = a.scat_cross_int + col * bandI;
    const double* mml = a.mmm_lay + (size_t)col * a.I;
    const double* mmi = a.mmm_int + (size_t)col * a.I;
    const size_t b = x + (size_t)a.X * i, k = c + nc * i;
    if (a.iso) {
        const double* pint = a.p_int + (size_t)col * a.I;
        const double ray = a.scat == 1 ? scl[b] : 0.0;
        a.dtau_u[col * nc * a.L + k] = (pint[i] - pint[i + 1]) / a.colpar[col].g * (opl[k] + ray / mml[i]);
        return;
    }
    double ray_up = 0, ray_low = 0;
    if (a.scat == 1) {
        ray_up = (scl[b] + sci[b + a.X]) / 2.0;
        ray_low = (sci[b] + scl[b]) / 2.0;
    }
    const double kap_up = (opl[k] + opi[k + nc]) / 2.0, kap_low = (opi[k] + opl[k]) / 2.0;
    const double mu_up = (mml[i] + mmi[i + 1]) / 2.0, mu_low = (mmi[i] + mml[i]) / 2.0;
    const size_t wgL = nc * a.L;
    a.dtau_u[col * wgL + k] = a.dcol_u[(size_t)col * a.L + i] * (kap_up + ray_up / mu_up);
    a.dtau_l[col * wgL + k] = a.dcol_l[(size_t)col * a.L + i] * (kap_low + ray_low / mu_low);
}
#endif

#ifndef HX_MATRIX_RCP
#define HX_MATRIX_RCP(x) newton_rcp(x)
#endif
__device__ __forceinline__ double newton_rcp(double x) {
    double r = __builtin_amdgcn_rcp(x);
    r = fma(fma(-x, r, 1.0), r, r);
    r = fma(fma(-x, r, 1.0), r, r);
    return r;
}

struct Moebius {
    double p11, p12, p21, p22;
};
__device__ __forceinline__ void moebius_after(Moebius& P, double q11, double q12, double q21, double q22) {
    const double n11 = fma(P.p11, q11, P.p12 * q21), n12 = fma(P.p11, q12, P.p12 * q22);
    const double n21 = fma(P.p21, q11, P.p22 * q21), n22 = fma(P.p21, q12, P.p22 * q22);
    P.p11 = n11; P.p12 = n12; P.p21 = n21; P.p22 = n22;
}
template <int CTRL, bool ONE>
__device__ __forceinline__ double dpp_or_identity(double v) {
    const int lo = __builtin_amdgcn_update_dpp(0, __double2loint(v), CTRL, 0xf, 0xf, true);
    const int hi = ONE ? __builtin_amdgcn_update_dpp(0x3FF00000, __double2hiint(v), CTRL, 0xf, 0xf, false)
                       : __builtin_amdgcn_update_dpp(0, __double2hiint(v), CTRL, 0xf, 0xf, true);
    return __hiloint2double(hi, lo);
}
template <int CTRL>
__device__ __forceinline__ void moebius_row_neighbour(Moebius& P) {
    moebius_after(P, dpp_or_identity<CTRL, true>(P.p11), dpp_or_identity<CTRL, false>(P.p12), dpp_or_identity<CTRL, false>(P.p21),
                  dpp_or_identity<CTRL, true>(P.p22));
}
template <int K>
__device__ __forceinline__ void moebius_scan_up(Moebius& P, int j, int k) {
    if (K) {
        moebius_row_neighbour<0x111>(P);
        moebius_row_neighbour<0x112>(P);
        moebius_row_neighbour<0x114>(P);
        moebius_row_neighbour<0x118>(P);
        if (K == 32 || K == 64) {
            const double q11 = dpp_move<0x142, 0xa>(P.p11), q12 = dpp_move<0x142, 0xa>(P.p12), q21 = dpp_move<0x142, 0xa>(P.p21),
                         q22 = dpp_move<0x142, 0xa>(P.p22);
            if (j & 16) moebius_after(P, q11, q12, q21, q22);
        }
        if (K == 64) {
            const double q11 = dpp_move<0x143, 0xc>(P.p11), q12 = dpp_move<0x143, 0xc>(P.p12), q21 = dpp_move<0x143, 0xc>(P.p21),
                         q22 = dpp_move<0x143, 0xc>(P.p22);
            if (j >= 32) moebius_after(P, q11, q12, q21, q22);
        }
    } else {
#define HX_MOEBIUS_STEP(N)                                                                                              \
    if (N < k) {                                                                                                        \
        const double q11 = from_lane_below<N>(P.p11, k), q12 = from_lane_below<N>(P.p12, k),                            \
                     q21 = from_lane_below<N>(P.p21, k), q22 = from_lane_below<N>(P.p22, k);                            \
        if (j >= N) moebius_after(P, q11, q12, q21, q22);                                                               \
    }
        HX_MOEBIUS_STEP(1) HX_MOEBIUS_STEP(2) HX_MOEBIUS_STEP(4) HX_MOEBIUS_STEP(8) HX_MOEBIUS_STEP(16) HX_MOEBIUS_STEP(32)
#undef HX_MOEBIUS_STEP
    }
}

#ifndef HX_BEAM_GROUP
#define HX_BEAM_GROUP 4
#endif
#ifndef HX_BIG_ROWS_ONE_WAVE
#define HX_BIG_ROWS_ONE_WAVE 1
#endif
constexpr bool flux_one_wave(int rows) { return rows >= 15 && HX_BIG_ROWS_ONE_WAVE; }
#define HX_FLUX_HEAD __global__ void __launch_bounds__(flux_one_wave(ROWS) ? 64 : 320) k_rt_flux(FluxArgs a)
#define HX_PLANE_T double
#define HX_PLANES a.coef
#include "rt_flux_kernel.inc"
#undef HX_FLUX_HEAD
#undef HX_PLANE_T
#undef HX_PLANES
#define HX_FLUX_HEAD __device__ __forceinline__ void rt_flux_f32_body(FluxArgs a, const float* coef32)
#define HX_PLANE_T float
#define HX_PLANES coef32
#include "rt_flux_kernel.inc"
#undef HX_FLUX_HEAD
#undef HX_PLANE_T
#undef HX_PLANES
template <int ROWS, int K = 0, bool MATRIX = false>
__global__ void __launch_bounds__(flux_one_wave(ROWS) ? 64 : 320) k_rt_flux_f32(FluxArgs a, const float* coef32) {
    rt_flux_f32_body<ROWS, K, MATRIX>(a, coef32);
}

#ifndef HX_PLANE_KERNELS_ONLY
__global__ void __launch_bounds__(256) k_rt_totals_a(KArgs a) {
    const int col = blockIdx.y, chunk = blockIdx.x;
    if (a.done[col]) return;
    const int I = a.I;
    const int per = (a.X + a.nchunk - 1) / a.nchunk;
    const int x0 = chunk * per, x1 = min(a.X, x0 + per);
    const double* __restrict__ fdir = a.F_dir_band_n + (size_t)col * a.X * I;
    const double* __restrict__ dl = a.deltawave;
    for (int t = threadIdx.x; t < 2 * I; t += blockDim.x) {
        const int dir = t / I, i = t - dir * I;
        const double* __restrict__ band = (dir == 0 ? a.F_down_band_n : a.F_up_band_n) + (size_t)col * a.X * I;
        double acc = 0.0;
        for (int xb = x0; xb < x1; xb += 8) {
            double v[8];
#pragma unroll
            for (int u = 0; u < 8; u++) {
                const int x = min(xb + u, x1 - 1);
                const double f = fdir[(size_t)x * I + i], b = band[(size_t)x * I + i];
                v[u] = dir == 0 ? f + b : b;
            }
#pragma unroll
            for (int u = 0; u < 8; u++)
                if (xb + u < x1) acc += v[u] * dl[xb + u];
        }
        a.tot_part[(((size_t)col * a.nchunk + chunk) * 2) * I + t] = acc;
    }
}

struct TotalsBArgs {
    KArgs a;
    RadTempArgs rt;
// ... 85 lines not shown
    const double *F_add_heat_sum, *F_smooth_sum;
    const double *F_down_tot, *F_up_tot, *F_net;
    int *conv_unstable, *conv_layer, *marked_red;
    const double* dampara;
    const int* done;
};

__device__ __forceinline__ ConvColumn conv_column(const ConvKArgs& a, int col) {
    const size_t L = a.L, I = a.L + 1;
    const hx_rt_column cp = a.colpar[col];
    ConvColumn c;
    c.T = a.T_lay + col * I;
    c.p_lay = a.p_lay + col * L;
    c.p_int = a.p_int + col * I;
    c.kappa_lay = a.kappa_lay + col * L;
    c.kappa_int = a.kappa_int + col * I;
    c.c_p = a.c_p + col * L;
    c.mmm = a.mmm_lay + col * I;
    c.F_add_heat_sum = a.F_add_heat_sum + col * L;
    c.F_smooth_sum = a.F_smooth_sum + col * L;
    c.F_down_tot = a.F_down_tot + col * I;
    c.F_up_tot = a.F_up_tot + col * I;
    c.F_net = a.F_net + col * I;
    c.conv_unstable = a.conv_unstable + col * I;
    c.conv_layer = a.conv_layer + col * I;
    c.marked_red = a.marked_red + col * I;
    c.L = a.L;
    c.itervalue = a.itervalue;
    c.F_intern = cp.F_intern;
    c.T_star = cp.T_star;
    c.dampara = a.dampara[col];
    c.rad_convergence_limit = cp.rad_convergence_limit;
    return c;
}

__global__ void __launch_bounds__(256) k_rt_conv_adjust(ConvKArgs a) {
    extern __shared__ __align__(16) double conv_smem[];
    __shared__ ConvTables t;
    const int col = blockIdx.x;
    if (a.done[col]) return;
    __shared__ ConvShared sh;
    ConvColumn c = conv_column(a, col), g;
    conv_stage_in(c, g, t, conv_smem, threadIdx.x, blockDim.x);
    convective_adjustment_wg(c, t, sh, threadIdx.x, blockDim.x);
    conv_stage_out(c, g, threadIdx.x, blockDim.x);
}

struct TotalsCArgs {
    KArgs a;
    ConvKArgs cv;
    ConvTempArgs ct;
    int* done_w;
    int* iters_done;
    int physical_tstep_on;
};

__global__ void __launch_bounds__(1024) k_rt_totals_c(TotalsCArgs q) {
    extern __shared__ __align__(16) double conv_smem[];
    __shared__ ConvTables t;
    __shared__ double seg[4][256];
    __shared__ int s_go;
    const KArgs& a = q.a;
    const int col = blockIdx.x;
    if (a.done[col]) return;
    const int I = a.I, L = a.L;
    double* up = a.F_up_tot + (size_t)col * I;
    double* down = a.F_down_tot + (size_t)col * I;
    double* net = a.F_net + (size_t)col * I;
    for (int t0 = 0; t0 < 2 * I; t0 += 256) {
        const int ts = t0 + (threadIdx.x & 255), sgm = threadIdx.x >> 8;
        const int cper = (a.nchunk + 3) / 4, c0 = sgm * cper, c1 = min(a.nchunk, c0 + cper);
        double s = 0.0;
        if (ts < 2 * I) {
            const double* __restrict__ part = a.tot_part + ((size_t)col * a.nchunk * 2) * I + ts;
            for (int cb = c0; cb < c1; cb += 8) {
                double v[8];
#pragma unroll
                for (int u = 0; u < 8; u++) v[u] = part[(size_t)min(cb + u, c1 - 1) * 2 * I];
#pragma unroll
                for (int u = 0; u < 8; u++)
                    if (cb + u < c1) s += v[u];
            }
        }
        seg[sgm][threadIdx.x & 255] = s;
        __syncthreads();
        if (sgm == 0 && ts < 2 * I) {
            const double tot = ((seg[0][threadIdx.x] + seg[1][threadIdx.x]) + seg[2][threadIdx.x]) + seg[3][threadIdx.x];
            if (ts < I) down[ts] = tot; else up[ts - I] = tot;
        }
        __syncthreads();
    }
    for (int i = threadIdx.x; i < I; i += blockDim.x) net[i] = up[i] - down[i];
    __syncthreads();
    ConvColumn c = conv_column(q.cv, col), g;
    conv_stage_in(c, g, t, conv_smem, threadIdx.x, blockDim.x);
    __shared__ ConvShared sh;
    __shared__ int s_convective;
    conv_find_lim(c, sh, threadIdx.x, blockDim.x);
    conv_mark_layers_wg(c, t, sh, 1, threadIdx.x, blockDim.x);
    int go = 0;
    if (!q.physical_tstep_on) {
        const int eq = conv_radiative_eq_wg(c, sh, &s_convective, threadIdx.x, blockDim.x);
        go = (!eq) || (c.itervalue < 400) || (s_convective == 0);
    }
    if (threadIdx.x == 0) {
        if (!go) {
            q.done_w[col] = 1;
            q.iters_done[col] = c.itervalue;
        }
        s_go = go;
    }
    __syncthreads();
    conv_stage_out(c, g, threadIdx.x, blockDim.x);
    __syncthreads();
    if (!s_go) return;
    const hx_rt_column cp = a.colpar[col];
    ConvTempArgs r = q.ct;
    r.F_net = net;
    r.F_net_diff += (size_t)col * L;
    r.tlay += (size_t)col * (L + 1);
    r.play += (size_t)col * L;
    r.pint += (size_t)col * I;
    r.T_store += (size_t)col * (L + 1);
    r.deltat_prefactor += (size_t)col * (L + 1);
    r.marked_red = g.marked_red;
    r.F_add_heat_lay += (size_t)col * L;
    r.F_smooth += (size_t)col * L;
    r.F_smooth_sum += (size_t)col * L;
    r.adapt_interval = cp.adapt_interval;
    r.F_intern = cp.F_intern;
    conv_temp_step(r, threadIdx.x, blockDim.x);
}

__global__ void k_rt_tint(const double* __restrict__ T_lay, double* __restrict__ T_int, int L, const int* done) {
    const int col = blockIdx.y, i = blockIdx.x * blockDim.x + threadIdx.x;
    if (i > L || done[col]) return;
    T_int[(size_t)col * (L + 1) + i] = interface_T(T_lay + (size_t)col * (L + 1), i, L);
}

__global__ void k_rt_heating(const double* __restrict__ dens, const double* __restrict__ dz,
                             double* __restrict__ F_lay, double* __restrict__ F_sum, int L, const int* done) {
    const int col = blockIdx.x;
    if (threadIdx.x != 0 || done[col]) return;
    dens += (size_t)col * L; dz += (size_t)col * L; F_lay += (size_t)col * L; F_sum += (size_t)col * L;
    double run = 0.0;
    for (int i = 0; i < L; i++) {
        const double f = dens[i] * dz[i];
        F_lay[i] = f;
        run = i == 0 ? f : run + f;
        F_sum[i] = run;
    }
}

__global__ void k_rt_height(const double* __restrict__ p_lay, const double* __restrict__ dz,
                            double* __restrict__ z, int L, int gas, size_t stride, const int* __restrict__ done) {
    const int col = blockIdx.x;
    p_lay += col * stride; dz += col * stride; z += col * stride;
    if (threadIdx.x != 0 || done[col]) return;
    if (gas) {
        int i0 = 0;
        for (int i = 0; i < L; i++) if (p_lay[i] >= 1e7) i0 = i;
        z[i0] = 0.0;
        for (int i = i0 + 1; i < L; i++) z[i] = z[i - 1] + 0.5 * dz[i - 1] + 0.5 * dz[i];
        for (int i = i0 - 1; i >= 0; i--) z[i] = z[i + 1] - 0.5 * dz[i + 1] - 0.5 * dz[i];
    } else {
        z[0] = 0.5 * dz[0];
        for (int i = 1; i < L; i++) z[i] = z[i - 1] + 0.5 * dz[i - 1] + 0.5 * dz[i];
    }
}

__global__ void k_rt_meanmolmass(const double* __restrict__ vmr, const double* __restrict__ weight,
                                 const int* __restrict__ in_mu, double* __restrict__ out, int nspecies,
                                 int nlev) {
    const int i = blockIdx.x * blockDim.x + threadIdx.x;
    if (i >= nlev) return;
    double num = 0.0, tot = 0.0;
    for (int s = 0; s < nspecies; s++)
        if (in_mu[s]) {
            num += vmr[(size_t)s * nlev + i] * weight[s];
            tot += vmr[(size_t)s * nlev + i];
        }
    out[i] = num / tot * HX_AMU;
}

__global__ void __launch_bounds__(256) k_rt_fdir_band(const double* __restrict__ F_dir_wg,
                                                      double* __restrict__ out,
                                                      const double* __restrict__ gauss_w, int X, int Y,
                                                      int I, const int* __restrict__ done) {
    __shared__ double tile[32][33];
    const int col = blockIdx.z;
    if (done[col]) return;
    const int x0 = blockIdx.x * 32, i0 = blockIdx.y * 32, tx = threadIdx.x & 31, ty = threadIdx.x >> 5;
    F_dir_wg += (size_t)col * Y * X * I;
    out += (size_t)col * X * I;
    for (int lv = ty; lv < 32; lv += 8) {
        const int x = x0 + tx, i = i0 + lv;
        double s = 0.0;
        if (x < X && i < I) {
            const double* f = F_dir_wg + (size_t)Y * x + (size_t)Y * X * i;
            if (Y == 20) {
                double v[20];
#pragma unroll
                for (int y = 0; y < 20; y += 2) {
                    const double2 p = *(const double2*)(f + y);
                    v[y] = p.x;
                    v[y + 1] = p.y;
                }
#pragma unroll
                for (int y = 0; y < 20; y++) s += 0.5 * gauss_w[y] * v[y];
            } else {
                for (int y = 0; y < Y; y++) s += 0.5 * gauss_w[y] * f[y];
            }
        }
        tile[lv][tx] = s;
    }
    __syncthreads();
    for (int xx = ty; xx < 32; xx += 8) {
        const int x = x0 + xx, i = i0 + tx;
        if (x < X && i < I) out[(size_t)x * I + i] = tile[tx][xx];
    }
}

__global__ void k_rt_tp_index(KArgs a, TPIndex* tp_lay, TPIndex* tp_int) {
    const int col = blockIdx.y, i = blockIdx.x * blockDim.x + threadIdx.x;
    if (i >= a.I || a.done[col]) return;
    const double* T = a.T_lay + (size_t)col * (a.L + 1);
    tp_int[(size_t)col * a.I + i] = locate_tp(interface_T(T, i, a.L), a.p_int[(size_t)col * a.I + i], a.ktemp,
                                              a.ntemp, a.kpress, a.npress, true, false);
    if (i < a.L)
        tp_lay[(size_t)col * a.I + i] = locate_tp(T[i], a.p_lay[(size_t)col * a.L + i], a.ktemp, a.ntemp, a.kpress,
                                                  a.npress, true, false);
}

__global__ void __launch_bounds__(256) k_rt_scat_interp(KArgs a, double* scat_lay, double* scat_int) {
    const int col = blockIdx.z, lev = blockIdx.y;
    const int x = blockIdx.x * blockDim.x + threadIdx.x;
    if (x >= a.X || a.done[col]) return;
    const size_t cp = a.X, ct = (size_t)a.X * a.npress, bandI = (size_t)a.X * a.I;
    const double* crosstable = a.coltab[col].scat_cross;
    for (int pass = 0; pass < 2; pass++) {
        if (pass == 0 && lev >= a.L) continue;
        const TPIndex k = (pass == 0 ? a.tp_lay : a.tp_int)[(size_t)col * a.I + lev];
        const double* t0 = crosstable + x + ct * k.tdown;
        const double* t1 = crosstable + x + ct * k.tup;
        (pass == 0 ? scat_lay : scat_int)[col * bandI + x + (size_t)a.X * lev] =
            blend_tp(t0[cp * k.pdown], t0[cp * k.pup], t1[cp * k.pdown], t1[cp * k.pup], k, false);
    }
}

__global__ void k_rt_mmm_table(KArgs a, double* mmm_lay, double* mmm_int) {
    const int col = blockIdx.y, i = blockIdx.x * blockDim.x + threadIdx.x;
    if (i >= a.I || a.done[col]) return;
    const double* __restrict__ table = a.coltab[col].meanmass;
    for (int pass = 0; pass < 2; pass++) {
        if (pass == 0 && i >= a.L) continue;
        const TPIndex k = (pass == 0 ? a.tp_lay : a.tp_int)[(size_t)col * a.I + i];
        (pass == 0 ? mmm_lay : mmm_int)[(size_t)col * a.I + i] =
            blend_tp(table[k.pdown + a.npress * k.tdown], table[k.pup + a.npress * k.tdown],
                     table[k.pdown + a.npress * k.tup], table[k.pup + a.npress * k.tup], k, false);
    }
}

__global__ void __launch_bounds__(256) k_rt_opac_table(KArgs a, double* opac_lay, double* opac_int) {
    const int col = blockIdx.z, lev = blockIdx.y;
    if (a.done[col]) return;
    const size_t nc = (size_t)a.Y * a.X, sp = nc, st = nc * a.npress, wgI = nc * a.I;
    const double* ktable = a.coltab[col].k;
    for (int pass = 0; pass < 2; pass++) {
        if (pass == 0 && lev >= a.L) continue;
        const TPIndex k = (pass == 0 ? a.tp_lay : a.tp_int)[(size_t)col * a.I + lev];
        double* out = (pass == 0 ? opac_lay : opac_int) + col * wgI + nc * lev;
        for (size_t c = (size_t)blockIdx.x * blockDim.x + threadIdx.x; c < nc; c += (size_t)gridDim.x * blockDim.x)
            out[c] = blend_tp(ktable[c + sp * k.pdown + st * k.tdown], ktable[c + sp * k.pup + st * k.tdown],
                              ktable[c + sp * k.pdown + st * k.tup], ktable[c + sp * k.pup + st * k.tup], k, false);
    }
}

__global__ void k_rt_delta_z(KArgs a, double* __restrict__ dz) {
    const int col = blockIdx.y, i = blockIdx.x * blockDim.x + threadIdx.x;
    if (i >= a.L || a.done[col]) return;
    const double* pint = a.p_int + (size_t)col * a.I;
    dz[(size_t)col * a.L + i] = HX_KBOLTZMANN * a.T_lay[(size_t)col * (a.L + 1) + i] /
                                (a.mmm_lay[(size_t)col * a.I + i] * a.colpar[col].g) * log(pint[i] / pint[i + 1]);
}

__global__ void __launch_bounds__(256) k_rt_total_g0(KArgs a, const double* __restrict__ g_cl_lay,
                                                     const double* __restrict__ g_cl_int, double* g_tot_lay,
                                                     double* g_tot_int) {
    const int col = blockIdx.z, lev = blockIdx.y;
    const int x = blockIdx.x * blockDim.x + threadIdx.x;
    if (x >= a.X || a.done[col]) return;
    const size_t k = (size_t)col * a.X * a.I + x + (size_t)a.X * lev;
    if (lev < a.L) {
        const double num = a.g_0 * a.scat_cross_lay[k] + g_cl_lay[k] * a.cl_sc_lay[k];
        g_tot_lay[k] = num / (a.scat_cross_lay[k] + a.cl_sc_lay[k]);
    }
    const double num = a.g_0 * a.scat_cross_int[k] + g_cl_int[k] * a.cl_sc_int[k];
    g_tot_int[k] = num / (a.scat_cross_int[k] + a.cl_sc_int[k]);
}

__global__ void k_rt_keep_ref_T(KArgs a, double* T_lay_ref, double* T_int_ref, TableSet* coltab_ref) {
    const int col = blockIdx.y, i = blockIdx.x * blockDim.x + threadIdx.x;
    if (a.done[col]) return;
    if (i == 0) coltab_ref[col] = a.coltab[col];
    if (i <= a.L) T_lay_ref[(size_t)col * (a.L + 1) + i] = a.T_lay[(size_t)col * (a.L + 1) + i];
    if (i < a.I) T_int_ref[(size_t)col * a.I + i] = a.T_int[(size_t)col * a.I + i];
}

__global__ void __launch_bounds__(256) k_rt_tile_rows(const double* __restrict__ src,
                                                      double* __restrict__ out, int X, int nlev) {
    const int x = blockIdx.x * blockDim.x + threadIdx.x, i = blockIdx.y;
    if (x < X) out[x + (size_t)X * i] = src[x];
}

#endif

bool coef_fp32_tiling(int rows, int k, bool generic_scans);
void launch_coef_f32(hx_rt* rt, const KArgs& a, int tpb, dim3 grid, size_t shmem);
void launch_flux_f32(hx_rt* rt, const FluxArgs& f, dim3 grid, size_t shmem);
hipError_t raise_flux_shmem_f32(hx_rt* rt, int shmem);
}
```

helios_amd/rt.py:

```python
import ctypes

import numpy as np

from . import _lib


class RtDims(ctypes.Structure):
    _fields_ = [("nbin", ctypes.c_int32), ("ny", ctypes.c_int32), ("nlayer", ctypes.c_int32),
                ("ncol", ctypes.c_int32), ("ntemp", ctypes.c_int32), ("npress", ctypes.c_int32),
                ("plancktable_dim", ctypes.c_int32), ("plancktable_step", ctypes.c_int32),
                ("nspecies", ctypes.c_int32), ("reserved", ctypes.c_int32 * 7)]


class RtFlags(ctypes.Structure):
    _fields_ = [("scat", ctypes.c_int32), ("dir_beam", ctypes.c_int32), ("clouds", ctypes.c_int32),
                ("scat_corr", ctypes.c_int32), ("geom_zenith_corr", ctypes.c_int32),
                ("smooth", ctypes.c_int32), ("real_star", ctypes.c_int32),
                ("planet_type_gas", ctypes.c_int32), ("kcoeff_mixing_ro", ctypes.c_int32),
                ("debug", ctypes.c_int32), ("iso", ctypes.c_int32), ("singlewalk", ctypes.c_int32),
                ("matrix", ctypes.c_int32), ("coef_fp32", ctypes.c_int32), ("reserved", ctypes.c_int32 * 2),
                ("epsi", ctypes.c_double), ("epsi2", ctypes.c_double), ("g_0", ctypes.c_double),
                ("i2s_transition", ctypes.c_double), ("w_0_limit", ctypes.c_double),
                ("w_0_scat_limit", ctypes.c_double), ("delta_tau_limit", ctypes.c_double),
                ("reserved_d", ctypes.c_double * 9)]
# ... 115 lines not shown
        arrs = [_f64(a) for a in (abs_lay, abs_int, scat_lay, scat_int, g0_lay, g0_int)]
        self._ck(self._l.hx_rt_set_column_clouds(self.handle, col, *[_dp(a) for a in arrs]),
                 "hx_rt_set_column_clouds")

    def add_mie_table(self, lamda_mie, scat, absorb):
        lam, sc, ab = _f64(lamda_mie), _f64(scat), _f64(absorb)
        if sc.ndim != 2 or sc.shape != ab.shape or sc.shape[1] != lam.size:
            raise ValueError("add_mie_table: scat %r and absorb %r must both be [nr][%d wavelengths]"
                             % (sc.shape, ab.shape, lam.size))
        idx = ctypes.c_int32(-1)
        self._ck(self._l.hx_rt_add_mie_table(self.handle, _dp(lam), int(lam.size), _dp(sc), _dp(ab), int(sc.shape[0]),
                                             ctypes.byref(idx)), "hx_rt_add_mie_table")
        return int(idx.value)

    def mie_table_count(self):
        return int(self.get("mie_table_count", -1)[0])

    def set_column_cloud_decks(self, col, mie_index, radius_weight, f_lay, f_int=None):
        idx = np.ascontiguousarray(mie_index, dtype=np.int32).reshape(-1)
        w, fl = np.atleast_2d(_f64(radius_weight)), np.atleast_2d(_f64(f_lay))
        fi = None if f_int is None else np.atleast_2d(_f64(f_int))
        nd = idx.size
        if w.shape[0] != nd or fl.shape != (nd, self.nlayer) or (fi is not None and fi.shape != (nd, self.ninterface)):
            raise ValueError("set_column_cloud_decks: %d decks need radius_weight [%d][nr], f_lay [%d][%d] and f_int [%d][%d]"
                             % (nd, nd, nd, self.nlayer, nd, self.ninterface))
        self._ck(self._l.hx_rt_set_column_cloud_decks(self.handle, int(col), nd, idx.ctypes.data_as(ctypes.POINTER(ctypes.c_int32)),
                                                      _dp(w), int(w.shape[1]), _dp(fl), _dp(fi)),
                 "hx_rt_set_column_cloud_decks")
        self._cloud_ndecks = nd

    def set_column_heating(self, col, F_add_heat_lay, F_add_heat_sum):
        a, b = _f64(F_add_heat_lay), _f64(F_add_heat_sum)
        self._ck(self._l.hx_rt_set_column_heating(self.handle, col, _dp(a), _dp(b)), "hx_rt_set_column_heating")

    def set_temperatures(self, col, T_lay):
        a = _f64(T_lay)
        self._ck(self._l.hx_rt_set_temperatures(self.handle, col, _dp(a)), "hx_rt_set_temperatures")

    def set_convergence_limit(self, col, limit):
        self._ck(self._l.hx_rt_set_convergence_limit(self.handle, col, float(limit)),
                 "hx_rt_set_convergence_limit")

    def set_state(self, col, name, array):
        a = np.ascontiguousarray(array)
        self._ck(self._l.hx_rt_set_state(self.handle, col, name.encode(), a.ctypes.data_as(ctypes.c_void_p),
                                         a.nbytes), "hx_rt_set_state(%s)" % name)

    def keep_down_fluxes(self, on=True):
        self.set_state(-1, "keep_down", np.array([1 if on else 0], np.int32))

    def build_planck_table(self, energy_correction=1):
        self._ck(self._l.hx_rt_build_planck_table(self.handle, int(energy_correction)),
                 "hx_rt_build_planck_table")

    def refresh(self):
        self._ck(self._l.hx_rt_refresh(self.handle), "hx_rt_refresh")

    def step(self, itervalue, step_temperature=True):
        self._ck(self._l.hx_rt_step(self.handle, int(itervalue), 1 if step_temperature else 0), "hx_rt_step")

    def run(self, itervalue, nsteps):
        self._ck(self._l.hx_rt_run(self.handle, int(itervalue), int(nsteps)), "hx_rt_run")

    def set_kappa_table(self, entr_temp, entr_press, entr_kappa, entr_c_p):
        a = [_f64(v) for v in (entr_temp, entr_press, entr_kappa, entr_c_p)]
        self._ck(self._l.hx_rt_set_kappa_table(self.handle, _dp(a[0]), len(a[0]), _dp(a[1]), len(a[1]), _dp(a[2]),
                                               _dp(a[3])), "hx_rt_set_kappa_table")

    def kappa_cp_refresh(self):
        self._ck(self._l.hx_rt_kappa_cp_refresh(self.handle), "hx_rt_kappa_cp_refresh")

    def conv_adjust(self, itervalue):
        self._ck(self._l.hx_rt_conv_adjust(self.handle, int(itervalue)), "hx_rt_conv_adjust")

    def conv_advance(self, itervalue):
        self._ck(self._l.hx_rt_conv_advance(self.handle, int(itervalue)), "hx_rt_conv_advance")

    def conv_run(self, itervalue, nsteps):
        self._ck(self._l.hx_rt_conv_run(self.handle, int(itervalue), int(nsteps)), "hx_rt_conv_run")

    def converged_layers(self):
        out = np.zeros(self.ncol, np.int32)
        self._ck(self._l.hx_rt_converged_layers(self.handle, out.ctypes.data_as(ctypes.POINTER(ctypes.c_int32))),
                 "hx_rt_converged_layers")
        return out

    _SHAPES = None

    def _shape(self, name):
        X, Y, L, I = self.nbin, self.ny, self.nlayer, self.ninterface
        wg = Y * X * I
        table = {
            "T_lay": (L + 1, np.float64), "T_int": (I, np.float64), "T_store": (L + 1, np.float64),
            "delta_t_prefactor": (L + 1, np.float64), "abort": (L + 1, np.int32),
            "F_up_band": (X * I, np.float64), "F_down_band": (X * I, np.float64),
            "F_dir_band": (X * I, np.float64), "F_up_tot": (I, np.float64), "F_down_tot": (I, np.float64),
            "F_net": (I, np.float64), "F_net_diff": (L, np.float64),
            "planckband_lay": (X * (L + 2), np.float64), "planckband_int": (X * I, np.float64),
            "opac_wg_lay": (Y * X * L, np.float64), "opac_wg_int": (wg, np.float64),
            "scat_cross_lay": (X * L, np.float64), "scat_cross_int": (X * I, np.float64),
            "meanmolmass_lay": (L, np.float64), "meanmolmass_int": (I, np.float64),
            "g_0_tot_lay": (X * L, np.float64), "g_0_tot_int": (X * I, np.float64),
            "delta_z_lay": (L, np.float64), "z_lay": (L, np.float64),
            "F_up_wg": (wg, np.float64), "F_down_wg": (wg, np.float64), "Fc_up_wg": (wg, np.float64),
            "Fc_down_wg": (wg, np.float64), "F_dir_wg": (wg, np.float64), "Fc_dir_wg": (wg, np.float64),
            "iters_done": (1, np.int32), "done": (1, np.int32), "premixed_table": (1, np.int32), "premixed_table_count": (1, np.int32), "flux_launch_policy": (2, np.float64), "graph_replays": (3, np.float64), "graph_builds": (2, np.float64),
            "conv_layer": (L + 1, np.int32), "conv_unstable": (L + 1, np.int32), "marked_red": (L + 1, np.int32),
            "kappa_lay": (L, np.float64), "kappa_int": (L + 1, np.float64), "c_p_lay": (L, np.float64),
            "F_smooth_sum": (L, np.float64), "F_add_heat_lay": (L, np.float64), "F_add_heat_sum": (L, np.float64),
            "planck_grid": ((self.dims.plancktable_dim + 1) * X, np.float64),
            "abs_cross_all_clouds_lay": (X * L, np.float64), "abs_cross_all_clouds_int": (X * I, np.float64),
            "scat_cross_all_clouds_lay": (X * L, np.float64), "scat_cross_all_clouds_int": (X * I, np.float64),
            "g_0_all_clouds_lay": (X * L, np.float64), "g_0_all_clouds_int": (X * I, np.float64),
            "cloud_deck_spectra": (max(1, getattr(self, "_cloud_ndecks", 0)) * 3 * X, np.float64),
            "mie_table_count": (1, np.int32),
            "vmr_lay": (max(1, self.dims.nspecies) * I, np.float64), "vmr_int": (max(1, self.dims.nspecies) * I, np.float64),
        }
        return table[name]

    def get(self, name, col=0):
        n, dt = self._shape(name)
        out = np.zeros(n, dt)
        self._ck(self._l.hx_rt_get(self.handle, int(col), name.encode(), out.ctypes.data_as(ctypes.c_void_p),
                                   out.nbytes), "hx_rt_get(%s)" % name)
        return out

    def device_ptr(self, name, col=0):
        p = ctypes.c_void_p()
        self._ck(self._l.hx_rt_device_ptr(self.handle, int(col), name.encode(), ctypes.byref(p)),
                 "hx_rt_device_ptr(%s)" % name)
        return p

    def traffic_model(self):
        v = [ctypes.c_double() for _ in range(4)]
        self._ck(self._l.hx_rt_traffic_model(self.handle, *[ctypes.byref(x) for x in v]), "hx_rt_traffic_model")
        return dict(step_algorithmic=v[0].value, step_actual=v[1].value,
                    refresh_algorithmic=v[2].value, refresh_actual=v[3].value)

    def profile(self, enable=True):
        self._ck(self._l.hx_rt_profile(self.handle, 1 if enable else 0), "hx_rt_profile")

    def profile_read(self, kernel):
        ms, n = ctypes.c_double(), ctypes.c_int()
        self._ck(self._l.hx_rt_profile_read(self.handle, kernel.encode(), ctypes.byref(ms), ctypes.byref(n)),
                 "hx_rt_profile_read")
        return ms.value, n.value

    def coef_plane_bytes(self):
        out = np.zeros(1, np.int32)
        self._ck(self._l.hx_rt_get(self.handle, -1, b"coef_plane_bytes", out.ctypes.data_as(ctypes.c_void_p), out.nbytes),
                 "hx_rt_get(coef_plane_bytes)")
        return int(out[0])

    _TILING = ("k", "ROWS", "threads", "nparts", "nxb", "ypb", "NW", "nplane", "has_vp", "pl_vp", "pl_dd", "coef_tpb",
               "coef_bytes", "generic_scans")

    def flux_tiling(self):
        out = np.zeros(len(self._TILING), np.int32)
        self._ck(self._l.hx_rt_get(self.handle, -1, b"flux_tiling", out.ctypes.data_as(ctypes.c_void_p), out.nbytes),
                 "hx_rt_get(flux_tiling)")
        return dict(zip(self._TILING, (int(v) for v in out)))

    def coef_planes(self, col=0):
        t = self.flux_tiling()
        dt = np.float32 if t["coef_bytes"] == 4 else np.float64
        per_tile = t["nplane"] * t["ROWS"] * 64
        ntiles = -(-self.nbin // t["nxb"]) * t["nparts"] * t["NW"]
        out = np.zeros(ntiles * per_tile, dt)
        self._ck(self._l.hx_rt_get(self.handle, int(col), b"coef_planes", out.ctypes.data_as(ctypes.c_void_p), out.nbytes),
                 "hx_rt_get(coef_planes)")
        return out.reshape(ntiles, t["nplane"], t["ROWS"], 64)

    def close(self):
        if self.handle:
            self._l.hx_rt_destroy(self.handle)
            self.handle = None


def case_flags(c):
    return dict(scat=int(c.scat), dir_beam=int(c.dir_beam), clouds=int(c.clouds),
                scat_corr=int(c.scat_corr), geom_zenith_corr=int(c.geom_zenith_corr),
                smooth=int(c.smooth), real_star=int(c.real_star),
                planet_type_gas=0 if c.get("planet_type", "gas") == "rocky" else 1,
                kcoeff_mixing_ro=0 if c.get("kcoeff_mixing", "RO") == "correlated-k" else 1, iso=int(c.get("iso", 0)),
                singlewalk=int(c.get("singlewalk", 0)), matrix=1 if c.get("flux_calc_method", "iteration") == "matrix" else 0,
                coef_fp32=1 if c.get("prec", "double") == "single" else 0,
                epsi=float(c.epsi), epsi2=float(c.epsi2), g_0=float(c.g_0),
                i2s_transition=float(c.i2s_transition), w_0_limit=float(c.w_0_limit),
                w_0_scat_limit=float(c.w_0_scat_limit), delta_tau_limit=float(c.delta_tau_limit))


def batch_from_case(ctx, c, ncol=1, nspecies=0, columns=None):
    flags = case_flags(c)
    col = dict(g=float(c.g), a=float(c.a), R_planet=float(c.R_planet), R_star=float(c.R_star),
               T_star=float(c.T_star), f_factor=float(c.f_factor), mu_star=float(c.mu_star),
               F_intern=float(c.F_intern), rad_convergence_limit=float(c.rad_convergence_limit),
               physical_tstep=float(c.physical_tstep), adapt_interval=int(c.adapt_interval),
               foreplay=int(c.foreplay), no_atmo=int(c.no_atmo))
    cols = [col] * ncol
    if columns is not None:
        cols = [dict(col, **{k: v for k, v in cp.items() if k in col}) for cp in columns]
    rt = RTBatch(ctx, c.nbin, c.ny, c.nlayer, ncol, c.ntemp, c.npress, c.plancktable_dim,
                 c.plancktable_step, flags, cols, nspecies=nspecies)
    try:
        rt.set_grid(c.opac_interwave, c.opac_deltawave, c.opac_wave, c.gauss_y, c.gauss_weight, c.ktemp, c.kpress)
        if nspecies == 0:
            if c.get("opac_k_factors") is not None:
                rt.set_premixed_separable(c.opac_k_factors[0], c.opac_k_factors[1], c.opac_scat_cross, c.opac_meanmass)
            else:
                rt.set_premixed_tables(c.opac_k, c.opac_scat_cross, c.opac_meanmass)
        rt.set_column_profile(-1, c.p_lay, c.p_int, c.T_lay, c.surf_albedo, c.starflux)
        if c.clouds:
            rt.set_column_clouds(-1, c.abs_cross_all_clouds_lay, c.abs_cross_all_clouds_int,
                                 c.scat_cross_all_clouds_lay, c.scat_cross_all_clouds_int,
                                 c.g_0_all_clouds_lay, c.g_0_all_clouds_int)
        rt.set_state(-1, "c_p_lay", np.asarray(c.c_p_lay, np.float64))
    except Exception:
        rt.close()
        raise
    return rt
```

Measured before the change: 2.511 billion bin*layer*iterations/s.

## Add specialized plain coef kernel and merge per-level refresh kernels

Adds a template-specialized coefficient kernel for the common no-cloud, no-beam, no-scattering-correction case. It precomputes ray/mu in shared memory and drops the beam, matrix-vote and vp/dd branches and stores. It also fuses tp_index, mmm_table, delta_z, height and keep_ref into one per-column refresh kernel to cut launches, and moves the coef launch dispatch into a separate translation unit with a one-time shared-memory attribute setup at init. The cost is more code paths, and the plain kernel needs extra shared memory for the rom image.

```diff
diff --git a/helios_amd/csrc/rt_coef.hip b/helios_amd/csrc/rt_coef.hip
--- /dev/null
+++ b/helios_amd/csrc/rt_coef.hip
@@ -0,0 +1,66 @@
+#define HX_PLANE_KERNELS_ONLY
+#include "rt_kernels.h"
+
+using namespace hx;
+
+namespace hx {
+
+namespace {
+
+template <int ROWS, int TPB, bool PLAIN>
+hipError_t coef_tpb(hx_rt* rt, const KArgs* a, dim3 grid, size_t shmem) {
+    const auto kernel = PLAIN ? k_rt_coef_plain<ROWS, TPB> : k_rt_coef<ROWS, TPB>;
+    if (!a) {
+        hipFuncAttributes attr;
+        return shmem > 64 * 1024 ? hipFuncSetAttribute((const void*)kernel, hipFuncAttributeMaxDynamicSharedMemorySize, (int)shmem)
+                                 : hipFuncGetAttributes(&attr, (const void*)kernel);
+    }
+    hipLaunchKernelGGL(kernel, grid, dim3(64 * TPB), shmem, rt->ctx->stream, *a);
+    return hipSuccess;
+}
+
+template <int ROWS, bool PLAIN>
+hipError_t coef_variant(hx_rt* rt, const KArgs* a, int tpb, dim3 grid, size_t shmem) {
+    switch (tpb) {
+        case 1: return coef_tpb<ROWS, 1, PLAIN>(rt, a, grid, shmem);
+        case 2: return coef_tpb<ROWS, 2, PLAIN>(rt, a, grid, shmem);
+        case 8:
+            if constexpr (ROWS <= 16) return coef_tpb<ROWS, 8, PLAIN>(rt, a, grid, shmem);
+            [[fallthrough]];
+        default: return coef_tpb<ROWS, 4, PLAIN>(rt, a, grid, shmem);
+    }
+}
+
+template <int ROWS>
+hipError_t coef_rows(hx_rt* rt, const KArgs* a, int tpb, dim3 grid, size_t shmem, bool plain) {
+    return plain ? coef_variant<ROWS, true>(rt, a, tpb, grid, shmem) : coef_variant<ROWS, false>(rt, a, tpb, grid, shmem);
+}
+
+}
+
+hipError_t launch_coef_f64(hx_rt* rt, const KArgs* a, int tpb, dim3 grid, size_t shmem, bool plain) {
+    switch (rt->g.ROWS) {
+        case 1: return coef_rows<1>(rt, a, tpb, grid, shmem, plain);
+        case 2: return coef_rows<2>(rt, a, tpb, grid, shmem, plain);
+        case 3: return coef_rows<3>(rt, a, tpb, grid, shmem, plain);
+        case 4: return coef_rows<4>(rt, a, tpb, grid, shmem, plain);
+        case 5: return coef_rows<5>(rt, a, tpb, grid, shmem, plain);
+        case 6: return coef_rows<6>(rt, a, tpb, grid, shmem, plain);
+        case 7: return coef_rows<7>(rt, a, tpb, grid, shmem, plain);
+        case 8: return coef_rows<8>(rt, a, tpb, grid, shmem, plain);
+        case 9: return coef_rows<9>(rt, a, tpb, grid, shmem, plain);
+        case 10: return coef_rows<10>(rt, a, tpb, grid, shmem, plain);
+        case 11: return coef_rows<11>(rt, a, tpb, grid, shmem, plain);
+        case 12: return coef_rows<12>(rt, a, tpb, grid, shmem, plain);
+        case 13: return coef_rows<13>(rt, a, tpb, grid, shmem, plain);
+        case 14: return coef_rows<14>(rt, a, tpb, grid, shmem, plain);
+        case 15: return coef_rows<15>(rt, a, tpb, grid, shmem, plain);
+        case 20: return coef_rows<20>(rt, a, tpb, grid, shmem, plain);
+        case 24: return coef_rows<24>(rt, a, tpb, grid, shmem, plain);
+        case 28: return coef_rows<28>(rt, a, tpb, grid, shmem, plain);
+        case 32: return coef_rows<32>(rt, a, tpb, grid, shmem, plain);
+        default: return coef_rows<16>(rt, a, tpb, grid, shmem, plain);
+    }
+}
+
+}
diff --git a/helios_amd/csrc/rt_coef_kernel.inc b/helios_amd/csrc/rt_coef_kernel.inc
--- a/helios_amd/csrc/rt_coef_kernel.inc
+++ b/helios_amd/csrc/rt_coef_kernel.inc
@@ -1,5 +1,5 @@
-template <int ROWS, int COEF_TPB>
-__global__ void __launch_bounds__(64 * COEF_TPB) HX_COEF_KERNEL(KArgs a HX_PLANE_ARG) {
+template <int ROWS, int COEF_TPB, bool PLAIN>
+__device__ __forceinline__ void HX_COEF_BODY(const KArgs& a HX_PLANE_ARG) {
     using CT = HX_PLANE_T;
     extern __shared__ __align__(16) double smem[];
     const int col = blockIdx.y;
@@ -14,8 +14,9 @@
     double* sh_ray = sh_int + (size_t)a.I * TSP;
     double* sh_mu = sh_ray + (size_t)a.H * NBX;
     double* sh_dc = sh_mu + a.H;
-    const size_t ncl = a.cloud_lds ? (size_t)a.H * NBX : 0;
-    double* sh_g0 = sh_dc + a.H;
+    const size_t ncl = !PLAIN && a.cloud_lds ? (size_t)a.H * NBX : 0;
+    double* sh_rom = sh_dc + a.H;
+    double* sh_g0 = sh_rom + (PLAIN ? (size_t)a.H * NBX : 0);
     double* sh_cab = sh_g0 + ncl;
     double* sh_csc = sh_cab + ncl;
     int* c_of_q = (int*)(sh_csc + ncl);
@@ -43,21 +44,27 @@
         const double* dcl = a.dcol_l + (size_t)col * a.L;
         const double* pint = a.p_int + (size_t)col * a.I;
         const double grav = a.colpar[col].g;
+        auto mu_of = [&](int h) -> double {
+            if (a.iso) return mml[h];
+            const int i = h >> 1, ii = i + (h & 1);
+            return (mmi[ii] + mml[i]) / 2.0;
+        };
         for (int h = threadIdx.x; h < a.H; h += blockDim.x) {
+            sh_mu[h] = mu_of(h);
             if (a.iso) {
-                sh_mu[h] = mml[h];
                 sh_dc[h] = (pint[h] - pint[h + 1]) / grav;
             } else {
-                const int i = h >> 1, ii = i + (h & 1);
-                sh_mu[h] = (mmi[ii] + mml[i]) / 2.0;
+                const int i = h >> 1;
                 sh_dc[h] = (h & 1) ? dcu[i] : dcl[i];
             }
         }
         for (int t = threadIdx.x; t < a.H * NBX; t += blockDim.x) {
             const int xs = t / a.H, h = t - xs * a.H, x = min(x_base + xs, a.X - 1);
             const size_t src = ((size_t)col * a.X + x) * a.H + h;
-            sh_ray[(size_t)h * NBX + xs] = a.half_ray[src];
-            if (a.cloud_lds) {
+            const double ray = a.half_ray[src];
+            sh_ray[(size_t)h * NBX + xs] = ray;
+            if constexpr (PLAIN) sh_rom[(size_t)h * NBX + xs] = ray / mu_of(h);
+            if (!PLAIN && a.cloud_lds) {
                 sh_g0[(size_t)h * NBX + xs] = a.half_g0[src];
                 sh_cab[(size_t)h * NBX + xs] = a.half_cab[src];
                 sh_csc[(size_t)h * NBX + xs] = a.half_csc[src];
@@ -126,9 +133,13 @@
         if (a.iso) return Fd[(size_t)c + nc * n];
         return (n & 1) ? Fc[(size_t)c + nc * (n >> 1)] : Fd[(size_t)c + nc * (n >> 1)];
     };
-    double F_here = beam_at_node(j * ROWS), F_above = beam_at_node(j * ROWS + 1);
+    double F_here = 0.0, F_above = 0.0;
+    if constexpr (!PLAIN) {
+        F_here = beam_at_node(j * ROWS);
+        F_above = beam_at_node(j * ROWS + 1);
+    }
     bool scatters = true;
-    if (a.matrix) {
+    if (!PLAIN && a.matrix) {
         bool mine = false;
 #pragma unroll 1
         for (int r = 0; r < ROWS; r++) {
@@ -162,8 +173,37 @@
         double alpha = 1.0, beta = 0.0, up = 0.0, vp = 0.0, dd = 0.0, du = 0.0;
         const double Fbot = F_here, Ftop = F_above;
         F_here = F_above;
-        F_above = beam_at_node(h + 2);
-        if (valid && h < a.H) {
+        if constexpr (!PLAIN) F_above = beam_at_node(h + 2);
+        if constexpr (PLAIN) {
+            if (valid && h < a.H) {
+                const int i = a.iso ? h : h >> 1;
+                const bool lower = a.iso || (h & 1) == 0;
+                const int ii = lower ? i : i + 1;
+                const double ray = sh_ray[(size_t)h * NBX + xs], rom = sh_rom[(size_t)h * NBX + xs];
+                const double o_l = sh_lay[(size_t)i * TSP + q], o_i = a.iso ? o_l : sh_int[(size_t)ii * TSP + q];
+                const double kap = a.iso ? o_l : (lower ? (o_i + o_l) / 2.0 : (o_l + o_i) / 2.0);
+                const double mu = sh_mu[h], dcol = sh_dc[h];
+                const double w0 = single_scat_albedo(ray, kap * mu, a.w_0_limit);
+                const double dtau = dcol * (kap + rom);
+                const Slab s = slab_coeffs_plain(w0, dtau, a.epsi);
+                const double invM = 1.0 / s.M;
+                alpha = s.P * invM;
+                beta = -s.N * invM;
+                const double K = 2.0 * HX_PI * a.epsi * (1.0 - w0) / (s.E - w0);
+                double u;
+                if (a.iso || dtau < a.dtau_limit) {
+                    u = (s.N + s.M - s.P) / 2.0;
+                } else {
+                    const double qq = a.epsi * (s.P - s.M + s.N) / dtau;
+                    u = (s.M + s.N) + qq;
+                }
+                up = K * u * invM;
+                if (h == 0) {
+                    a.boaK[col * nc + c] = (1.0 - w0) / (s.E - w0);
+                    a.Fdir0[col * nc + c] = 0.0;
+                }
+            }
+        } else if (valid && h < a.H) {
             const int i = a.iso ? h : h >> 1;
             const bool lower = a.iso || (h & 1) == 0;
             const int ii = lower ? i : i + 1;
@@ -233,16 +273,25 @@
             __builtin_nontemporal_store(alpha, ctile + 0 * ROWS * 64 + off);
             __builtin_nontemporal_store(beta, ctile + 1 * ROWS * 64 + off);
             __builtin_nontemporal_store(up, ctile + 2 * ROWS * 64 + off);
-            if (a.has_vp) __builtin_nontemporal_store(vp, ctile + (size_t)a.pl_vp * ROWS * 64 + off);
+            if (!PLAIN && a.has_vp) __builtin_nontemporal_store(vp, ctile + (size_t)a.pl_vp * ROWS * 64 + off);
         } else {
             __builtin_nontemporal_store(plane0_code(alpha, beta), ctile + 0 * ROWS * 64 + off);
             __builtin_nontemporal_store(plane1_code(beta), ctile + 1 * ROWS * 64 + off);
             __builtin_nontemporal_store((CT)up, ctile + 2 * ROWS * 64 + off);
-            if (a.has_vp) __builtin_nontemporal_store((CT)(up + vp), ctile + (size_t)a.pl_vp * ROWS * 64 + off);
-        }
-        if (a.dir_beam == 1) {
+            if (!PLAIN && a.has_vp) __builtin_nontemporal_store((CT)(up + vp), ctile + (size_t)a.pl_vp * ROWS * 64 + off);
+        }
+        if (!PLAIN && a.dir_beam == 1) {
             __builtin_nontemporal_store((CT)dd, ctile + (size_t)a.pl_dd * ROWS * 64 + off);
             __builtin_nontemporal_store((CT)du, ctile + (size_t)(a.pl_dd + 1) * ROWS * 64 + off);
         }
     }
 }
+
+template <int ROWS, int COEF_TPB>
+__global__ void __launch_bounds__(64 * COEF_TPB) HX_COEF_KERNEL(KArgs a HX_PLANE_ARG) {
+    HX_COEF_BODY<ROWS, COEF_TPB, false>(a HX_PLANE_PASS);
+}
+template <int ROWS, int COEF_TPB>
+__global__ void __launch_bounds__(64 * COEF_TPB) HX_COEF_KERNEL_PLAIN(KArgs a HX_PLANE_ARG) {
+    HX_COEF_BODY<ROWS, COEF_TPB, true>(a HX_PLANE_PASS);
+}
diff --git a/helios_amd/csrc/rt_fused.h b/helios_amd/csrc/rt_fused.h
--- a/helios_amd/csrc/rt_fused.h
+++ b/helios_amd/csrc/rt_fused.h
@@ -65,7 +65,8 @@
     double state_cache_mb = 0;
     bool generic_scans = false;
     bool conv_shmem_raised = false;
-    bool coef_shmem_raised = false;
+    bool coef_plain = false;
+    bool refresh_split = false;
 
     double *interwave = nullptr, *deltawave = nullptr, *wave = nullptr, *gauss_y = nullptr,
            *gauss_w = nullptr, *ktemp = nullptr, *kpress = nullptr;
diff --git a/helios_amd/csrc/rt_fused.hip b/helios_amd/csrc/rt_fused.hip
--- a/helios_amd/csrc/rt_fused.hip
+++ b/helios_amd/csrc/rt_fused.hip
@@ -294,46 +294,32 @@
     DISPATCH_ROWS(flux_rows, rt, &f);
 }
 
-template <int ROWS, int TPB>
-void launch_coef_tpb(hx_rt* rt, KArgs a) {
-    const TileGeom& g = rt->g;
-    const int ntiles = g.nblk_x * g.nparts * g.NW;
-    const int TS = TPB * g.S, TSP = TS;
-    const int NBX = g.nxb * ((TPB - 1) / (g.NW * g.nparts) + 2);
-    a.coef_nbx = NBX;
-    size_t shmem = ((size_t)(rt->L + rt->I) * TSP + (size_t)rt->H * (NBX + 2)) * sizeof(double) + 2 * TS * sizeof(int);
-    const size_t cloud_image = 3 * (size_t)rt->H * NBX * sizeof(double);
-    a.cloud_lds = a.clouds == 1 && rt->cloud_lds && shmem + cloud_image <= 80 * 1024;
-    if (a.cloud_lds) shmem += cloud_image;
-    if (rt->coef32) {
-        launch_coef_f32(rt, a, TPB, dim3((ntiles + TPB - 1) / TPB, rt->C), shmem);
-        return;
-    }
-    if (shmem > 64 * 1024 && !rt->coef_shmem_raised) {
-        (void)hipFuncSetAttribute((const void*)k_rt_coef<ROWS, TPB>, hipFuncAttributeMaxDynamicSharedMemorySize,
-                                  (int)shmem);
-        rt->coef_shmem_raised = true;
-    }
-    hipLaunchKernelGGL(HIP_KERNEL_NAME(k_rt_coef<ROWS, TPB>), dim3((ntiles + TPB - 1) / TPB, rt->C), dim3(64 * TPB),
-                       shmem, rt->ctx->stream, a);
-}
-template <int ROWS>
-void launch_coef(hx_rt* rt, const KArgs& a) {
-    switch (rt->coef_tpb) {
-        case 1: launch_coef_tpb<ROWS, 1>(rt, a); break;
-        case 2: launch_coef_tpb<ROWS, 2>(rt, a); break;
-        case 8:
-            if constexpr (ROWS <= 16) { launch_coef_tpb<ROWS, 8>(rt, a); break; }
-            [[fallthrough]];
-        default: launch_coef_tpb<ROWS, 4>(rt, a); break;
-    }
-}
-
 size_t coef_shmem_bytes(const hx_rt* rt, int tpb) {
     const TileGeom& g = rt->g;
     const int TS = tpb * g.S;
     const int NBX = g.nxb * ((tpb - 1) / (g.NW * g.nparts) + 2);
-    return ((size_t)(rt->L + rt->I) * TS + (size_t)rt->H * (NBX + 2)) * sizeof(double) + 2 * TS * sizeof(int);
+    return ((size_t)(rt->L + rt->I) * TS + (size_t)rt->H * (NBX + 2 + (rt->coef_plain ? NBX : 0))) * sizeof(double) +
+           2 * TS * sizeof(int);
+}
+
+hipError_t launch_coef(hx_rt* rt, const KArgs* args) {
+    const TileGeom& g = rt->g;
+    const int TPB = rt->coef_tpb;
+    const int ntiles = g.nblk_x * g.nparts * g.NW;
+    const int NBX = g.nxb * ((TPB - 1) / (g.NW * g.nparts) + 2);
+    size_t shmem = coef_shmem_bytes(rt, TPB);
+    const size_t cloud_image = 3 * (size_t)rt->H * NBX * sizeof(double);
+    const bool cloud_lds = rt->f.clouds == 1 && rt->cloud_lds && shmem + cloud_image <= 80 * 1024;
+    if (cloud_lds) shmem += cloud_image;
+    const dim3 grid((ntiles + TPB - 1) / TPB, rt->C);
+    KArgs a;
+    if (args) {
+        a = *args;
+        a.coef_nbx = NBX;
+        a.cloud_lds = cloud_lds ? 1 : 0;
+    }
+    if (rt->coef_bytes == 4) return launch_coef_f32(rt, args ? &a : nullptr, TPB, grid, shmem, rt->coef_plain);
+    return launch_coef_f64(rt, args ? &a : nullptr, TPB, grid, shmem, rt->coef_plain);
 }
 
 int set_flux_shmem_limits(hx_rt* rt) {
@@ -410,6 +396,9 @@
     if (const char* e = getenv("HELIOS_RT_CLOUD_LDS")) rt->cloud_lds = atoi(e) != 0;
     rt->coef_tpb = std::max(1, std::min(8, 16 / std::max(1, rt->g.S)));
     if (const char* e = getenv("HELIOS_RT_COEF_TPB")) rt->coef_tpb = atoi(e);
+    rt->coef_plain = flags->clouds != 1 && flags->scat_corr != 1 && flags->g_0 == 0.0 && flags->dir_beam != 1 && !rt->matrix;
+    if (const char* e = getenv("HELIOS_RT_COEF_GENERAL")) rt->coef_plain = rt->coef_plain && atoi(e) == 0;
+    if (const char* e = getenv("HELIOS_RT_REFRESH_SPLIT")) rt->refresh_split = atoi(e) != 0;
     if (rt->coef_tpb != 1 && rt->coef_tpb != 2 && !(rt->coef_tpb == 8 && rt->g.ROWS <= 16)) rt->coef_tpb = 4;
     while (rt->coef_tpb > 1 && coef_shmem_bytes(rt, rt->coef_tpb) > 150 * 1024) rt->coef_tpb /= 2;
     if (coef_shmem_bytes(rt, rt->coef_tpb) > 160 * 1024)
@@ -426,6 +415,7 @@
     rt->species.resize(dims->nspecies > 0 ? dims->nspecies : 0);
     int rc = set_flux_shmem_limits(rt);
     if (rc) return rc;
+    HX_HIP(ctx, launch_coef(rt, nullptr));
 
     const size_t X = rt->X, Y = rt->Y, L = rt->L, I = rt->I, C = rt->C, nc = X * Y;
     RT_ALLOC(rt->interwave, X + 1); RT_ALLOC(rt->deltawave, X); RT_ALLOC(rt->wave, X);
@@ -974,13 +964,23 @@
     bool fused_lookup = rt->d.nspecies == 0 && !rt->f.dir_beam;
     if (const char* e = getenv("HELIOS_RT_FUSED_LOOKUP")) fused_lookup = fused_lookup && atoi(e) != 0;
     rt->opac_stale = fused_lookup;
+    const bool levels_merged = rt->d.nspecies == 0 && !rt->refresh_split;
+    const bool ray_in_half_bands = levels_merged && !rt->f.clouds && !rt->f.dir_beam;
     if (rt->d.nspecies == 0) {
-        k_rt_tp_index<<<dim3(hx_cdiv(I, 64), C), 64, 0, ctx->stream>>>(a, (TPIndex*)rt->tp_lay, (TPIndex*)rt->tp_int);
-        k_rt_scat_interp<<<dim3(hx_cdiv(X, 256), I, C), 256, 0, ctx->stream>>>(a, rt->scat_cross_lay, rt->scat_cross_int);
-        k_rt_mmm_table<<<dim3(hx_cdiv(I, 64), C), 64, 0, ctx->stream>>>(a, rt->mmm_lay, rt->mmm_int);
+        if (levels_merged) {
+            RefreshLevelsOut o = {(TPIndex*)rt->tp_lay, (TPIndex*)rt->tp_int, rt->mmm_lay, rt->mmm_int, rt->delta_z, rt->z_lay,
+                                  rt->T_lay_ref, rt->T_int_ref, rt->coltab_ref, fused_lookup ? 1 : 0, rt->f.planet_type_gas};
+            k_rt_refresh_levels<<<C, 256, 2 * (size_t)L * sizeof(double), ctx->stream>>>(a, o);
+        } else {
+            k_rt_tp_index<<<dim3(hx_cdiv(I, 64), C), 64, 0, ctx->stream>>>(a, (TPIndex*)rt->tp_lay, (TPIndex*)rt->tp_int);
+        }
+        if (!ray_in_half_bands)
+            k_rt_scat_interp<<<dim3(hx_cdiv(X, 256), I, C), 256, 0, ctx->stream>>>(a, rt->scat_cross_lay, rt->scat_cross_int);
+        if (!levels_merged) k_rt_mmm_table<<<dim3(hx_cdiv(I, 64), C), 64, 0, ctx->stream>>>(a, rt->mmm_lay, rt->mmm_int);
         HX_LAUNCH_CHECK(ctx);
         if (fused_lookup) {
-            k_rt_keep_ref_T<<<dim3(hx_cdiv(I + 1, 64), C), 64, 0, ctx->stream>>>(a, rt->T_lay_ref, rt->T_int_ref, rt->coltab_ref);
+            if (!levels_merged)
+                k_rt_keep_ref_T<<<dim3(hx_cdiv(I + 1, 64), C), 64, 0, ctx->stream>>>(a, rt->T_lay_ref, rt->T_int_ref, rt->coltab_ref);
         } else {
             ProfScope ps(rt, "opac_interpol");
             const int chunks = (int)std::min<long long>(hx_cdiv((long long)nc, 256), 1024);
@@ -996,9 +996,11 @@
                                                                           rt->g0_tot_lay, rt->g0_tot_int);
         HX_LAUNCH_CHECK(ctx);
     }
-    k_rt_delta_z<<<dim3(hx_cdiv(L, 64), C), 64, 0, ctx->stream>>>(a, rt->delta_z);
-    k_rt_height<<<C, 64, 0, ctx->stream>>>(rt->p_lay, rt->delta_z, rt->z_lay, L, rt->f.planet_type_gas, (size_t)L, rt->done);
-    HX_LAUNCH_CHECK(ctx);
+    if (!levels_merged) {
+        k_rt_delta_z<<<dim3(hx_cdiv(L, 64), C), 64, 0, ctx->stream>>>(a, rt->delta_z);
+        k_rt_height<<<C, 64, 0, ctx->stream>>>(rt->p_lay, rt->delta_z, rt->z_lay, L, rt->f.planet_type_gas, (size_t)L, rt->done);
+        HX_LAUNCH_CHECK(ctx);
+    }
     if (rt->has_heating) {
         k_rt_heating<<<C, 64, 0, ctx->stream>>>(rt->add_heat_dens, rt->delta_z, rt->F_add_heat_lay,
                                                 rt->F_add_heat_sum, L, rt->done);
@@ -1018,10 +1020,12 @@
     }
     {
         ProfScope ps(rt, "rt_coef");
-        k_rt_half_bands<<<dim3(hx_cdiv(X, 32), hx_cdiv(rt->H, 32), C), 256, 0, ctx->stream>>>(a);
+        const dim3 grid_half(hx_cdiv(X, 32), hx_cdiv(rt->H, 32), C);
+        if (ray_in_half_bands) k_rt_half_bands_ray<<<grid_half, 256, 0, ctx->stream>>>(a, rt->scat_cross_lay, rt->scat_cross_int);
+        else k_rt_half_bands<<<grid_half, 256, 0, ctx->stream>>>(a);
         HX_LAUNCH_CHECK(ctx);
         a.from_table = fused_lookup ? 1 : 0;
-        DISPATCH_ROWS(launch_coef, rt, a);
+        (void)launch_coef(rt, &a);
         HX_LAUNCH_CHECK(ctx);
     }
     rt->refreshed = true;
@@ -1486,6 +1490,12 @@
     if (strcmp(name, "coef_plane_bytes") == 0) {
         HX_REQUIRE(rt->ctx, out_bytes == sizeof(int32_t), HX_E_ARG, "coef_plane_bytes is one int32");
         const int32_t v = rt->coef_bytes;
+        memcpy(out, &v, sizeof(v));
+        return 0;
+    }
+    if (strcmp(name, "coef_kernel_plain") == 0) {
+        HX_REQUIRE(rt->ctx, out_bytes == sizeof(int32_t), HX_E_ARG, "coef_kernel_plain is one int32");
+        const int32_t v = rt->coef_plain ? 1 : 0;
         memcpy(out, &v, sizeof(v));
         return 0;
     }
diff --git a/helios_amd/csrc/rt_fused_f32.hip b/helios_amd/csrc/rt_fused_f32.hip
--- a/helios_amd/csrc/rt_fused_f32.hip
+++ b/helios_amd/csrc/rt_fused_f32.hip
@@ -11,25 +11,33 @@
 
 namespace {
 
-template <int ROWS, int TPB>
-void coef_tpb(hx_rt* rt, const KArgs& a, dim3 grid, size_t shmem) {
-    if (shmem > 64 * 1024 && !rt->coef_shmem_raised) {
-        (void)hipFuncSetAttribute((const void*)k_rt_coef_f32<ROWS, TPB>, hipFuncAttributeMaxDynamicSharedMemorySize,
-                                  (int)shmem);
-        rt->coef_shmem_raised = true;
+template <int ROWS, int TPB, bool PLAIN>
+hipError_t coef_tpb(hx_rt* rt, const KArgs* a, dim3 grid, size_t shmem) {
+    const auto kernel = PLAIN ? k_rt_coef_plain_f32<ROWS, TPB> : k_rt_coef_f32<ROWS, TPB>;
+    if (!a) {
+        hipFuncAttributes attr;
+        return shmem > 64 * 1024 ? hipFuncSetAttribute((const void*)kernel, hipFuncAttributeMaxDynamicSharedMemorySize, (int)shmem)
+                                 : hipFuncGetAttributes(&attr, (const void*)kernel);
     }
-    hipLaunchKernelGGL(HIP_KERNEL_NAME(k_rt_coef_f32<ROWS, TPB>), grid, dim3(64 * TPB), shmem, rt->ctx->stream, a,
-                       rt->coef32);
+    hipLaunchKernelGGL(kernel, grid, dim3(64 * TPB), shmem, rt->ctx->stream, *a, rt->coef32);
+    return hipSuccess;
+}
+
+template <int ROWS, bool PLAIN>
+hipError_t coef_variant(hx_rt* rt, const KArgs* a, int tpb, dim3 grid, size_t shmem) {
+    switch (tpb) {
+        case 1: return coef_tpb<ROWS, 1, PLAIN>(rt, a, grid, shmem);
+        case 2: return coef_tpb<ROWS, 2, PLAIN>(rt, a, grid, shmem);
+        case 8:
+            if constexpr (ROWS <= 16) return coef_tpb<ROWS, 8, PLAIN>(rt, a, grid, shmem);
+            [[fallthrough]];
+        default: return coef_tpb<ROWS, 4, PLAIN>(rt, a, grid, shmem);
+    }
 }
 
 template <int ROWS>
-void coef_rows(hx_rt* rt, const KArgs& a, int tpb, dim3 grid, size_t shmem) {
-    switch (tpb) {
-        case 1: coef_tpb<ROWS, 1>(rt, a, grid, shmem); break;
-        case 2: coef_tpb<ROWS, 2>(rt, a, grid, shmem); break;
-        case 8: coef_tpb<ROWS, 8>(rt, a, grid, shmem); break;
-        default: coef_tpb<ROWS, 4>(rt, a, grid, shmem); break;
-    }
+hipError_t coef_rows(hx_rt* rt, const KArgs* a, int tpb, dim3 grid, size_t shmem, bool plain) {
+    return plain ? coef_variant<ROWS, true>(rt, a, tpb, grid, shmem) : coef_variant<ROWS, false>(rt, a, tpb, grid, shmem);
 }
 
 template <int ROWS, int K, bool MATRIX>
@@ -81,8 +89,8 @@
 
 }
 
-void launch_coef_f32(hx_rt* rt, const KArgs& a, int tpb, dim3 grid, size_t shmem) {
-    F32_DISPATCH_ROWS(coef_rows, a, tpb, grid, shmem);
+hipError_t launch_coef_f32(hx_rt* rt, const KArgs* a, int tpb, dim3 grid, size_t shmem, bool plain) {
+    F32_DISPATCH_ROWS(coef_rows, a, tpb, grid, shmem, plain);
 }
 
 void launch_flux_f32(hx_rt* rt, const FluxArgs& f, dim3 grid, size_t shmem) {
diff --git a/helios_amd/csrc/rt_kernels.h b/helios_amd/csrc/rt_kernels.h
--- a/helios_amd/csrc/rt_kernels.h
+++ b/helios_amd/csrc/rt_kernels.h
@@ -351,25 +351,82 @@
     }
 }
 
+__device__ __forceinline__ double scat_at(const double* crosstable, int x, int X, int npress, const TPIndex& k) {
+    const size_t cp = X, ct = (size_t)X * npress;
+    const double* t0 = crosstable + x + ct * k.tdown;
+    const double* t1 = crosstable + x + ct * k.tup;
+    return blend_tp(t0[cp * k.pdown], t0[cp * k.pup], t1[cp * k.pdown], t1[cp * k.pup], k, false);
+}
+
+__global__ void __launch_bounds__(256) k_rt_half_bands_ray(KArgs a, double* scat_lay, double* scat_int) {
+    __shared__ double s_lay[32][33], s_int[33][33], tile[32][33];
+    const int col = blockIdx.z;
+    if (a.done[col]) return;
+    const int tx = threadIdx.x & 31, ty = threadIdx.x >> 5;
+    const size_t bandI = (size_t)a.X * a.I;
+    const double* crosstable = a.coltab[col].scat_cross;
+    const int h0 = blockIdx.y * 32;
+    const int lo = a.iso ? h0 : h0 >> 1, nown = a.iso ? 32 : 16;
+    const int x = blockIdx.x * 32 + tx;
+    for (int sl = ty; sl <= nown; sl += 8) {
+        const int lev = lo + sl;
+        if (x >= a.X || lev >= a.I) continue;
+        const double vi = scat_at(crosstable, x, a.X, a.npress, a.tp_int[(size_t)col * a.I + lev]);
+        s_int[sl][tx] = vi;
+        if (sl < nown || lev == a.I - 1) scat_int[col * bandI + x + (size_t)a.X * lev] = vi;
+        if (sl < nown && lev < a.L) {
+            const double vl = scat_at(crosstable, x, a.X, a.npress, a.tp_lay[(size_t)col * a.I + lev]);
+            s_lay[sl][tx] = vl;
+            scat_lay[col * bandI + x + (size_t)a.X * lev] = vl;
+        }
+    }
+    __syncthreads();
+    for (int hh = ty; hh < 32; hh += 8) {
+        const int h = h0 + hh;
+        if (x < a.X && h < a.H) {
+            const int i = a.iso ? h : h >> 1, ii = a.iso ? h : i + (h & 1);
+            tile[hh][tx] = a.scat != 1 ? 0.0 : a.iso ? s_lay[i - lo][tx] : (s_int[ii - lo][tx] + s_lay[i - lo][tx]) / 2.0;
+        }
+    }
+    __syncthreads();
+    const int h = h0 + tx;
+    for (int xx = ty; xx < 32; xx += 8) {
+        const int xo = blockIdx.x * 32 + xx;
+        if (xo < a.X && h < a.H) a.half_ray[((size_t)col * a.X + xo) * a.H + h] = tile[tx][xx];
+    }
+}
+
 #endif
 
 #define HX_COEF_KERNEL k_rt_coef
+#define HX_COEF_KERNEL_PLAIN k_rt_coef_plain
+#define HX_COEF_BODY rt_coef_body
 #define HX_PLANE_T double
 #define HX_PLANE_ARG
+#define HX_PLANE_PASS
 #define HX_PLANES a.coef
 #include "rt_coef_kernel.inc"
 #undef HX_COEF_KERNEL
+#undef HX_COEF_KERNEL_PLAIN
+#undef HX_COEF_BODY
 #undef HX_PLANE_T
 #undef HX_PLANE_ARG
+#undef HX_PLANE_PASS
 #undef HX_PLANES
 #define HX_COEF_KERNEL k_rt_coef_f32
+#define HX_COEF_KERNEL_PLAIN k_rt_coef_plain_f32
+#define HX_COEF_BODY rt_coef_body_f32
 #define HX_PLANE_T float
 #define HX_PLANE_ARG , float* coef32
+#define HX_PLANE_PASS , coef32
 #define HX_PLANES coef32
 #include "rt_coef_kernel.inc"
 #undef HX_COEF_KERNEL
+#undef HX_COEF_KERNEL_PLAIN
+#undef HX_COEF_BODY
 #undef HX_PLANE_T
 #undef HX_PLANE_ARG
+#undef HX_PLANE_PASS
 #undef HX_PLANES
 
 #ifndef HX_PLANE_KERNELS_ONLY
@@ -761,11 +818,7 @@
     }
 }
 
-__global__ void k_rt_height(const double* __restrict__ p_lay, const double* __restrict__ dz,
-                            double* __restrict__ z, int L, int gas, size_t stride, const int* __restrict__ done) {
-    const int col = blockIdx.x;
-    p_lay += col * stride; dz += col * stride; z += col * stride;
-    if (threadIdx.x != 0 || done[col]) return;
+__device__ __forceinline__ void height_walk(const double* p_lay, const double* dz, double* __restrict__ z, int L, int gas) {
     if (gas) {
         int i0 = 0;
         for (int i = 0; i < L; i++) if (p_lay[i] >= 1e7) i0 = i;
@@ -776,6 +829,14 @@
         z[0] = 0.5 * dz[0];
         for (int i = 1; i < L; i++) z[i] = z[i - 1] + 0.5 * dz[i - 1] + 0.5 * dz[i];
     }
+}
+
+__global__ void k_rt_height(const double* __restrict__ p_lay, const double* __restrict__ dz,
+                            double* __restrict__ z, int L, int gas, size_t stride, const int* __restrict__ done) {
+    const int col = blockIdx.x;
+    p_lay += col * stride; dz += col * stride; z += col * stride;
+    if (threadIdx.x != 0 || done[col]) return;
+    height_walk(p_lay, dz, z, L, gas);
 }
 
 __global__ void k_rt_meanmolmass(const double* __restrict__ vmr, const double* __restrict__ weight,
@@ -830,31 +891,35 @@
     }
 }
 
+__device__ __forceinline__ TPIndex level_tp(const KArgs& a, int col, int i, bool lay) {
+    const double* T = a.T_lay + (size_t)col * (a.L + 1);
+    if (lay) return locate_tp(T[i], a.p_lay[(size_t)col * a.L + i], a.ktemp, a.ntemp, a.kpress, a.npress, true, false);
+    return locate_tp(interface_T(T, i, a.L), a.p_int[(size_t)col * a.I + i], a.ktemp, a.ntemp, a.kpress, a.npress, true, false);
+}
+
 __global__ void k_rt_tp_index(KArgs a, TPIndex* tp_lay, TPIndex* tp_int) {
     const int col = blockIdx.y, i = blockIdx.x * blockDim.x + threadIdx.x;
     if (i >= a.I || a.done[col]) return;
-    const double* T = a.T_lay + (size_t)col * (a.L + 1);
-    tp_int[(size_t)col * a.I + i] = locate_tp(interface_T(T, i, a.L), a.p_int[(size_t)col * a.I + i], a.ktemp,
-                                              a.ntemp, a.kpress, a.npress, true, false);
-    if (i < a.L)
-        tp_lay[(size_t)col * a.I + i] = locate_tp(T[i], a.p_lay[(size_t)col * a.L + i], a.ktemp, a.ntemp, a.kpress,
-                                                  a.npress, true, false);
+    tp_int[(size_t)col * a.I + i] = level_tp(a, col, i, false);
+    if (i < a.L) tp_lay[(size_t)col * a.I + i] = level_tp(a, col, i, true);
 }
 
 __global__ void __launch_bounds__(256) k_rt_scat_interp(KArgs a, double* scat_lay, double* scat_int) {
     const int col = blockIdx.z, lev = blockIdx.y;
     const int x = blockIdx.x * blockDim.x + threadIdx.x;
     if (x >= a.X || a.done[col]) return;
-    const size_t cp = a.X, ct = (size_t)a.X * a.npress, bandI = (size_t)a.X * a.I;
+    const size_t bandI = (size_t)a.X * a.I;
     const double* crosstable = a.coltab[col].scat_cross;
     for (int pass = 0; pass < 2; pass++) {
         if (pass == 0 && lev >= a.L) continue;
         const TPIndex k = (pass == 0 ? a.tp_lay : a.tp_int)[(size_t)col * a.I + lev];
-        const double* t0 = crosstable + x + ct * k.tdown;
-        const double* t1 = crosstable + x + ct * k.tup;
-        (pass == 0 ? scat_lay : scat_int)[col * bandI + x + (size_t)a.X * lev] =
-            blend_tp(t0[cp * k.pdown], t0[cp * k.pup], t1[cp * k.pdown], t1[cp * k.pup], k, false);
-    }
+        (pass == 0 ? scat_lay : scat_int)[col * bandI + x + (size_t)a.X * lev] = scat_at(crosstable, x, a.X, a.npress, k);
+    }
+}
+
+__device__ __forceinline__ double mmm_at(const double* __restrict__ table, int npress, const TPIndex& k) {
+    return blend_tp(table[k.pdown + npress * k.tdown], table[k.pup + npress * k.tdown], table[k.pdown + npress * k.tup],
+                    table[k.pup + npress * k.tup], k, false);
 }
 
 __global__ void k_rt_mmm_table(KArgs a, double* mmm_lay, double* mmm_int) {
@@ -864,9 +929,7 @@
     for (int pass = 0; pass < 2; pass++) {
         if (pass == 0 && i >= a.L) continue;
         const TPIndex k = (pass == 0 ? a.tp_lay : a.tp_int)[(size_t)col * a.I + i];
-        (pass == 0 ? mmm_lay : mmm_int)[(size_t)col * a.I + i] =
-            blend_tp(table[k.pdown + a.npress * k.tdown], table[k.pup + a.npress * k.tdown],
-                     table[k.pdown + a.npress * k.tup], table[k.pup + a.npress * k.tup], k, false);
+        (pass == 0 ? mmm_lay : mmm_int)[(size_t)col * a.I + i] = mmm_at(table, a.npress, k);
     }
 }
 
@@ -885,12 +948,16 @@
     }
 }
 
+__device__ __forceinline__ double layer_height(double T, double mmm, double grav, double p_bot, double p_top) {
+    return HX_KBOLTZMANN * T / (mmm * grav) * log(p_bot / p_top);
+}
+
 __global__ void k_rt_delta_z(KArgs a, double* __restrict__ dz) {
     const int col = blockIdx.y, i = blockIdx.x * blockDim.x + threadIdx.x;
     if (i >= a.L || a.done[col]) return;
     const double* pint = a.p_int + (size_t)col * a.I;
-    dz[(size_t)col * a.L + i] = HX_KBOLTZMANN * a.T_lay[(size_t)col * (a.L + 1) + i] /
-                                (a.mmm_lay[(size_t)col * a.I + i] * a.colpar[col].g) * log(pint[i] / pint[i + 1]);
+    dz[(size_t)col * a.L + i] = layer_height(a.T_lay[(size_t)col * (a.L + 1) + i], a.mmm_lay[(size_t)col * a.I + i],
+                                             a.colpar[col].g, pint[i], pint[i + 1]);
 }
 
 __global__ void __launch_bounds__(256) k_rt_total_g0(KArgs a, const double* __restrict__ g_cl_lay,
@@ -908,12 +975,54 @@
     g_tot_int[k] = num / (a.scat_cross_int[k] + a.cl_sc_int[k]);
 }
 
+__device__ __forceinline__ void keep_ref_level(const KArgs& a, int col, int i, double* T_lay_ref, double* T_int_ref,
+                                               TableSet* coltab_ref) {
+    if (i == 0) coltab_ref[col] = a.coltab[col];
+    if (i <= a.L) T_lay_ref[(size_t)col * (a.L + 1) + i] = a.T_lay[(size_t)col * (a.L + 1) + i];
+    if (i < a.I) T_int_ref[(size_t)col * a.I + i] = a.T_int[(size_t)col * a.I + i];
+}
+
 __global__ void k_rt_keep_ref_T(KArgs a, double* T_lay_ref, double* T_int_ref, TableSet* coltab_ref) {
     const int col = blockIdx.y, i = blockIdx.x * blockDim.x + threadIdx.x;
     if (a.done[col]) return;
-    if (i == 0) coltab_ref[col] = a.coltab[col];
-    if (i <= a.L) T_lay_ref[(size_t)col * (a.L + 1) + i] = a.T_lay[(size_t)col * (a.L + 1) + i];
-    if (i < a.I) T_int_ref[(size_t)col * a.I + i] = a.T_int[(size_t)col * a.I + i];
+    keep_ref_level(a, col, i, T_lay_ref, T_int_ref, coltab_ref);
+}
+
+struct RefreshLevelsOut {
+    TPIndex *tp_lay, *tp_int;
+    double *mmm_lay, *mmm_int, *delta_z, *z_lay, *T_lay_ref, *T_int_ref;
+    TableSet* coltab_ref;
+    int keep_ref, gas;
+};
+__global__ void __launch_bounds__(256) k_rt_refresh_levels(KArgs a, RefreshLevelsOut o) {
+    extern __shared__ __align__(16) double smem[];
+    const int col = blockIdx.x;
+    if (a.done[col]) return;
+    double* sh_p = smem;
+    double* sh_dz = smem + a.L;
+    const double* __restrict__ table = a.coltab[col].meanmass;
+    const double* pint = a.p_int + (size_t)col * a.I;
+    const double grav = a.colpar[col].g;
+    for (int i = threadIdx.x; i < a.I; i += blockDim.x) {
+        if (i < a.I) {
+            const TPIndex ki = level_tp(a, col, i, false);
+            o.tp_int[(size_t)col * a.I + i] = ki;
+            o.mmm_int[(size_t)col * a.I + i] = mmm_at(table, a.npress, ki);
+        }
+        if (i < a.L) {
+            const TPIndex kl = level_tp(a, col, i, true);
+            o.tp_lay[(size_t)col * a.I + i] = kl;
+            const double mmm = mmm_at(table, a.npress, kl);
+            o.mmm_lay[(size_t)col * a.I + i] = mmm;
+            const double dz = layer_height(a.T_lay[(size_t)col * (a.L + 1) + i], mmm, grav, pint[i], pint[i + 1]);
+            o.delta_z[(size_t)col * a.L + i] = dz;
+            sh_dz[i] = dz;
+            sh_p[i] = a.p_lay[(size_t)col * a.L + i];
+        }
+        if (o.keep_ref) keep_ref_level(a, col, i, o.T_lay_ref, o.T_int_ref, o.coltab_ref);
+    }
+    __syncthreads();
+    if (threadIdx.x == 0) height_walk(sh_p, sh_dz, o.z_lay + (size_t)col * a.L, a.L, o.gas);
 }
 
 __global__ void __launch_bounds__(256) k_rt_tile_rows(const double* __restrict__ src,
@@ -925,7 +1034,8 @@
 #endif
 
 bool coef_fp32_tiling(int rows, int k, bool generic_scans);
-void launch_coef_f32(hx_rt* rt, const KArgs& a, int tpb, dim3 grid, size_t shmem);
+hipError_t launch_coef_f32(hx_rt* rt, const KArgs* a, int tpb, dim3 grid, size_t shmem, bool plain);
+hipError_t launch_coef_f64(hx_rt* rt, const KArgs* a, int tpb, dim3 grid, size_t shmem, bool plain);
 void launch_flux_f32(hx_rt* rt, const FluxArgs& f, dim3 grid, size_t shmem);
 hipError_t raise_flux_shmem_f32(hx_rt* rt, int shmem);
 }
diff --git a/helios_amd/rt.py b/helios_amd/rt.py
--- a/helios_amd/rt.py
+++ b/helios_amd/rt.py
@@ -291,6 +291,12 @@
                  "hx_rt_get(coef_plane_bytes)")
         return int(out[0])
 
+    def coef_kernel_plain(self):
+        out = np.zeros(1, np.int32)
+        self._ck(self._l.hx_rt_get(self.handle, -1, b"coef_kernel_plain", out.ctypes.data_as(ctypes.c_void_p), out.nbytes),
+                 "hx_rt_get(coef_kernel_plain)")
+        return bool(out[0])
+
     _TILING = ("k", "ROWS", "threads", "nparts", "nxb", "ypb", "NW", "nplane", "has_vp", "pl_vp", "pl_dd", "coef_tpb",
                "coef_bytes", "generic_scans")
 
```

Measured after the change: 2.542 billion bin*layer*iterations/s, median of 6. 1.01x the previous value.
